# rdesc/autorally

Hardware: AMD Instinct MI355X
Metric: trajectory rollouts/s per MPPI solve (higher is better)
Workload: dtype f32

## Files before the change

autorally_amd/build.py:

```python
import os
import shutil
import subprocess
import sys
from concurrent.futures import ThreadPoolExecutor

HERE = os.path.dirname(os.path.abspath(__file__))
CSRC = os.path.join(HERE, "csrc")
LIB = os.path.join(HERE, "libmppi_hip.so")
SOURCES = ["mppi_abi.hip", "abi_forms.hip", "abi_pack.hip", "abi_solve.hip", "abi_host.hip", "abi_trace.hip", "rollout_mfma.hip", "rollout_multi.hip", "rollout_oct.hip", "rollout_row.hip", "rollout_row64.hip", "rollout_m44.hip", "rollout_lds44.hip", "rollout_lds128.hip", "rollout_lds16.hip", "rollout_fleet16.hip", "rollout_fleet_multi.hip", "rollout_glb16.hip", "rollout_glb44.hip", "rollout_valu.hip", "rollout_trace.hip", "ddp_fleet.hip", "nominal_fleet.hip", "solve_kernels.hip",
           "noise_mrg32k3a.hip", "rollout_bf.hip", "rollout_bf_row.hip", "ddp_feedback.cpp"]
HEADERS = ["abi_internal.hpp", "mppi_device.hpp", "mfma_net.hpp", "group_roles.hpp", "m44_core.hpp", "m44_group.hpp", "multi_group.hpp", "wave16_step.hpp", "wave16_image.hpp", "mppi_kernels.hpp", "noise_device.hpp", "ddp_feedback.hpp", "basis_funcs.hpp", "bf_device.hpp", "bf_row_device.hpp", "host_net.hpp", "tanhf_vec.hpp", "tanhf_scalar.hpp", "ddp_fleet_device.hpp", os.path.join("..", "..", "include", "mppi_hip.h")]
FLAGS = ["--offload-arch=gfx950", "-O3", "-ffp-contract=off", "-fPIC", "-std=c++17", "-Wall",
         "-Wno-unused-function", "-mllvm", "-amdgpu-mfma-vgpr-form", "-Xarch_host", "-mavx2", "-Xarch_host", "-mfma"]


EXTRA_FLAGS = {"rollout_row.hip": ["-mllvm", "-amdgpu-sched-strategy=max-ilp"],
               "rollout_row64.hip": ["-mllvm", "-amdgpu-sched-strategy=max-ilp"]}


def hipcc():
    for c in (os.environ.get("HIPCC"), shutil.which("hipcc"), "/opt/rocm/bin/hipcc"):
        if c and os.path.exists(c):
            return c
    raise RuntimeError("hipcc not found")


def _stale(target, deps):
    if not os.path.exists(target):
        return True
    t = os.path.getmtime(target)
    return any(os.path.getmtime(d) > t for d in deps)


def build(force=False, verbose=False):
    cc = hipcc()
    objdir = os.path.join(HERE, "build")
    os.makedirs(objdir, exist_ok=True)
    hdrs = [os.path.join(CSRC, h) for h in HEADERS]
    if not force and not _stale(LIB, [os.path.join(CSRC, s) for s in SOURCES] + hdrs):
        return LIB
    jobs = []
    objs = []
    for s in SOURCES:
        src = os.path.join(CSRC, s)
        obj = os.path.join(objdir, s.replace(".hip", ".o").replace(".cpp", ".o"))
        objs.append(obj)
        if force or _stale(obj, [src] + hdrs):
            jobs.append([cc] + FLAGS + EXTRA_FLAGS.get(s, []) + ["-c", src, "-o", obj])

    def run(cmd):
        if verbose:
            print(" ".join(cmd), file=sys.stderr)
        r = subprocess.run(cmd, capture_output=True, text=True)
        if r.returncode != 0:
            raise RuntimeError("hipcc failed:\n%s\n%s" % (" ".join(cmd), r.stderr))
        return r.stderr

    with ThreadPoolExecutor(max_workers=4) as ex:
        for warn in ex.map(run, jobs):
            if verbose and warn:
                print(warn, file=sys.stderr)
    if jobs or force or _stale(LIB, objs):
        run([cc, "--offload-arch=gfx950", "-shared", "-fPIC", "-o", LIB] + objs)
    return LIB


HOST = os.path.join(HERE, "host")
BIN = os.path.join(HERE, "bin")


def build_host(force=False):
    os.makedirs(BIN, exist_ok=True)
    cxx = shutil.which("g++") or "g++"
    hdrs = [os.path.join(HOST, h) for h in ("npz.hpp", "param_getter.hpp", "mppi_controller_hip.hpp",
                                            "run_control_loop.hpp", "path_integral_main.hpp")] + [os.path.join(CSRC, h) for h in ("basis_funcs.hpp", "host_net.hpp", "tanhf_vec.hpp")] + [os.path.join(HERE, "..", "include", "mppi_hip.h")]
    outs = []
    link = ["-L" + HERE, "-lmppi_hip", "-Wl,-rpath,$ORIGIN/.."]
    for name, libs in (("host_selftest", link), ("path_integral_nn", link), ("path_integral_bf", link)):
        src = os.path.join(HOST, name + ".cpp")
        out = os.path.join(BIN, name)
        outs.append(out)
        if force or _stale(out, [src] + hdrs + ([LIB] if libs else [])):
            cmd = [cxx, "-O2", "-mavx2", "-mfma", "-ffp-contract=off", "-std=c++17", "-Wall", "-DMPPI_NPZ_ZLIB", src, "-o", out] + libs + ["-lz", "-lpthread"]
            r = subprocess.run(cmd, capture_output=True, text=True)
            if r.returncode != 0:
                raise RuntimeError("host build failed:\n%s\n%s" % (" ".join(cmd), r.stderr))
    return outs


if __name__ == "__main__":
    print(build(force="--force" in sys.argv, verbose=True))
    print(build_host(force="--force" in sys.argv))
```

autorally_amd/csrc/abi_internal.hpp:

```cpp
#pragma once
#include "../../include/mppi_hip.h"

#include <hip/hip_runtime.h>

#include <chrono>
#include <cmath>
#include <cstdio>
#include <cstdlib>
#include <cstring>
#include <atomic>
#include <condition_variable>
#include <functional>
#include <mutex>
#include <new>
#include <thread>
#include <string>
#include <vector>

#include "mppi_kernels.hpp"
#include "ddp_feedback.hpp"
#include "basis_funcs.hpp"
#include "host_net.hpp"

namespace mppi_abi {
// ... 51 lines not shown
  NetDesc net{};
  bool mfma_ok = false;
  int hidden = 0, n_hidden = 0;
  mppi_abi::Pref pref = mppi_abi::Pref::Auto;
  mppi_abi::Form forced = mppi_abi::Form::Auto;
  bool multi_standalone_noise = false;
  int num_simds = 1024;
  hipStream_t stream = nullptr;
  hipStream_t order_stream = nullptr;
  int n_slots = 1;
  bool u_dirty = true;
  unsigned seq = 0;
  std::vector<float> sg_buf;
  bool basis = false;
  float ddp_Q[7] = {0.5f, 0.5f, 0.25f, 0.0f, 0.05f, 0.01f, 0.01f};
  float ddp_R[2] = {10.0f, 10.0f};
  float ddp_Qf[7] = {0, 0, 0, 0, 0, 0, 0};
  DdpResult ddp;
  bool have_ddp = false;
  int ddp_on_device = 0;
  int nominal_on_device = 0;
  hipStream_t batch_s = nullptr;
  unsigned *d_counter = nullptr;
  float *d_part = nullptr;
  unsigned long long *d_gx = nullptr;
  unsigned long long *d_min_cost = nullptr;
  unsigned min_cost_tag = 0;
  bool use_min_cost = true;
  unsigned long long *d_ug = nullptr;
  unsigned tail_epoch = 0, tail_poll_ticks = 2000000;
  float *d_res_map = nullptr;

  std::vector<float> U, hist, theta, map_rgba;
  HostNetFma hnet;
  int map_w = 0, map_h = 0;
  mppi_cost_params cost{};
  float r_c1[3] = {0, 0, 0}, r_c2[3] = {0, 0, 0}, trs[3] = {0, 0, 1};
  float u_lo[2] = {0, 0}, u_hi[2] = {0, 0};
  bool have_nn = false, have_map = false, have_cost = false;

  float *d_in = nullptr, *d_scal = nullptr;
  float *d_in_buf[2] = {nullptr, nullptr};
  int in_cur = 0;
  bool slid_valid = false;
  float *d_noise = nullptr, *d_stage = nullptr;
  float *d_gen[2] = {nullptr, nullptr};
  int gen_cur = 0;
  bool gen_async = false;
  bool prefetch_valid = false;
  float *v_buf = nullptr;
  hipStream_t gstream = nullptr;
  hipEvent_t ev_gen = nullptr, ev_s1 = nullptr;
  hipEvent_t ev_gt[2] = {nullptr, nullptr};
  bool gen_timed = false, gen_time_now = false;
  float *d_costs = nullptr, *d_w = nullptr;
  float *d_theta = nullptr, *d_wpack = nullptr, *d_map = nullptr;
  float *d_theta_s = nullptr;
  float *d_rowpack = nullptr;
  float *d_bfrowpack = nullptr;
  float *d_row64pack = nullptr;
  float *d_m44pack = nullptr;
  float *d_lds44pack = nullptr;
  float *d_lds128pack = nullptr;
  size_t lds128_bytes = 0;
  float *d_lds16pack = nullptr;
  size_t lds16_bytes = 0;
  mppi_abi::ArgBlock *fleet_one = nullptr;
  float *d_glb16pack = nullptr;
  size_t glb16_bytes = 0;
  int glb16_cap = -1;
  float *d_glb44pack = nullptr;
  size_t glb44_bytes = 0;
  int glb44_cap = -1;
  float *d_tracepack = nullptr;
  float *d_trace = nullptr;
  int *h_trace_ks = nullptr, *d_trace_ks = nullptr;
  int trace_chunk = 0;
  float solve_state[7] = {0, 0, 0, 0, 0, 0, 0};
  bool have_solve = false;
  bool have_weights = false;
  bool valu_reg_ok = false;
  double *d_invt = nullptr;
  uint32_t *d_rng[2] = {nullptr, nullptr};
  uint32_t *d_jump = nullptr, *d_sub = nullptr, *d_one = nullptr;
  int rng_cur = 0;
  int noise_L = 1, noise_C = 1;
  float *h_in = nullptr, *h_res = nullptr;
  int explicit_iters = 0;
  bool pending = false;
  bool pending_timed = false;
  bool pending_armed = false;
  float traj_cost = 0.0f, baseline = 0.0f, eta = 0.0f;

  int spin_budget = 0, fault_wave = 0;
  float *d_cap = nullptr;
  bool capture = false, cap_valid = false, cap_explicit = false;
  double wait_timeout_s = 30.0;
  unsigned *gate_cpu = nullptr, *d_gate = nullptr;
  bool gate_bar = false;
  bool chain = true;
  int gate_blk = 0;
  int armed = 0;
  unsigned arm_seq = 0;
  unsigned seq_floor = 0;
  int arm_in = 0;
  float *arm_vbuf = nullptr;
  bool arm_publish_only = false;
  int arm_n = 0;
  mppi_handle *arm_peers[4] = {nullptr, nullptr, nullptr, nullptr};
  hipStream_t arm_stream = nullptr;
  hipEvent_t ev_arm = nullptr;
  std::chrono::steady_clock::time_point arm_until;
  float *d_costs_alt = nullptr, *d_w_alt = nullptr;
  int launch_instances = 0;
  bool launch_gated = false;
  bool timed_out = false;
  bool no_result = false;
  bool timing = false;
  int timing_every = 1;
  unsigned timing_count = 0;
  std::vector<Events> ev;
  mppi_stage_times acc{};
  std::string err;
};

namespace mppi_abi {
using namespace mppi;


#define HIPCHK(h, call)                                                  \
  do {                                                                   \
    hipError_t e__ = (call);                                             \
    if (e__ != hipSuccess) return fail((h), MPPI_ERR_HIP, #call, e__);   \
  } while (0)
inline hipError_t ensure_device(int dev)
{
  int cur = -1;
  if (hipGetDevice(&cur) == hipSuccess && cur == dev) return hipSuccess;
  return hipSetDevice(dev);
}
#define OWN(h)                      \
  do {                              \
    int rc__ = own_stream(h);       \
    if (rc__) return rc__;          \
  } while (0)

int compute_k99(int K);
std::vector<float> pack_mfma_weights(const std::vector<float> &theta, int H, int NHID);
std::vector<float> pack_row_weights(const std::vector<float> &theta);
std::vector<float> pack_bf_row_weights(const std::vector<float> &W);
std::vector<float> pack_row64_weights(const std::vector<float> &theta, int NHID);
std::vector<float> pack_m44_weights(const std::vector<float> &theta, int NHID);
std::vector<float> pack_lds44_weights(const std::vector<float> &theta, const mppi::NetDesc &net);
std::vector<float> pack_lds128_weights(const std::vector<float> &theta, const mppi::NetDesc &net);
std::vector<float> pack_lds16_weights(const std::vector<float> &theta, const mppi::NetDesc &net);
std::vector<float> pack_glb16_weights(const std::vector<float> &theta, const mppi::NetDesc &net);
int upload_glb16_image(mppi_handle *h);
std::vector<float> pack_glb44_weights(const std::vector<float> &theta, const mppi::NetDesc &net);
int upload_glb44_image(mppi_handle *h);
std::vector<float> pack_trace_weights(const std::vector<float> &theta, const mppi::NetDesc &net);
int seed_device(mppi_handle *h, uint64_t seed, uint64_t offset);
int upload_rng_tables(mppi_handle *h);
bool use_mfma(const mppi_handle *h);
bool use_valu_reg(const mppi_handle *h);
Form form_of(const mppi_handle *h);
bool form_generator_noise(const mppi_handle *h);
// ... 62 lines not shown
```

autorally_amd/csrc/abi_pack.hip:

```cpp
#include "abi_internal.hpp"

using namespace mppi;
using namespace mppi_abi;

namespace mppi_abi {

constexpr uint64_t M1 = 4294967087ULL, M2 = 4294944443ULL;

struct Mat3 {
  uint32_t a[9];
};
Mat3 mat_mul(const Mat3 &A, const Mat3 &B, uint64_t m)
{
  Mat3 R;
  for (int i = 0; i < 3; i++)
    for (int j = 0; j < 3; j++) {
      uint64_t acc = 0;
      for (int k = 0; k < 3; k++) acc = (acc + (uint64_t)A.a[3 * i + k] * B.a[3 * k + j] % m) % m;
      R.a[3 * i + j] = (uint32_t)acc;
    }
  return R;
}
Mat3 mat_identity()
{
  Mat3 R{{1, 0, 0, 0, 1, 0, 0, 0, 1}};
  return R;
}
Mat3 mat_pow(Mat3 A, uint64_t e, uint64_t m)
{
  Mat3 R = mat_identity();
  while (e) {
    if (e & 1) R = mat_mul(R, A, m);
    A = mat_mul(A, A, m);
    e >>= 1;
  }
  return R;
}
Mat3 base_A1() { return Mat3{{0, 1, 0, 0, 0, 1, (uint32_t)(M1 - 810728ULL), 1403580u, 0}}; }
Mat3 base_A2() { return Mat3{{0, 1, 0, 0, 0, 1, (uint32_t)(M2 - 1370589ULL), 0, 527612u}}; }

int compute_k99(int K)
{
  const double thr = .99 * (double)K;
  int k = 0;
  while (k < K && !((double)k >= thr)) k++;
  return k;
}

std::vector<float> pack_mfma_weights(const std::vector<float> &theta, int H, int NHID)
{
  const int MT = H / 16, KSH = H / 4;
  const int nA0 = MT * 2, nAH = MT * KSH, nAL = KSH;
  const int nA = nA0 + (NHID - 1) * nAH + nAL;
  const int nBias = NHID * MT * 4 + 4;
  const int nTree = 4 * KSH + 1;
  std::vector<float> out((size_t)(nA + nBias + nTree) * 64, 0.0f);
  std::vector<int> wo, bo, nin, nout;
  int off = 0, prev = kNetIn;
  for (int l = 0; l <= NHID; l++) {
    const int no = (l < NHID) ? H : kNetOut;
    wo.push_back(off);
    bo.push_back(off + no * prev);
    nin.push_back(prev);
    nout.push_back(no);
    off += no * prev + no;
    prev = no;
  }
  for (int lane = 0; lane < 64; lane++) {
    const int row = lane & 15, kk = lane >> 4;
    const int gq = row >> 2, rq = row & 3;
    for (int m = 0; m < MT; m++)
      for (int s = 0; s < 2; s++) {
        const int n = 16 * m + 4 * rq + gq, kap = 4 * s + kk;
        out[(size_t)(m * 2 + s) * 64 + lane] = (kap < kNetIn) ? theta[wo[0] + n * kNetIn + kap] : 0.0f;
      }
    for (int l = 1; l < NHID; l++) {
      const int aoff = nA0 + (l - 1) * nAH;
      for (int m = 0; m < MT; m++)
        for (int s = 0; s < KSH; s++) {
          const int n = 16 * m + 4 * rq + gq, kap = 4 * s + kk;
          out[(size_t)(aoff + m * KSH + s) * 64 + lane] = theta[wo[l] + n * H + kap];
        }
    }
    {
      const int aoff = nA0 + (NHID - 1) * nAH;
      for (int s = 0; s < KSH; s++) {
        const int o = row & 3, kap = 4 * s + kk;
        out[(size_t)(aoff + s) * 64 + lane] = theta[wo[NHID] + o * H + kap];
      }
    }
    const int g = lane >> 4;
    for (int l = 0; l < NHID; l++)
      for (int m = 0; m < MT; m++)
        for (int r = 0; r < 4; r++)
          out[(size_t)(nA + l * MT * 4 + m * 4 + r) * 64 + lane] = theta[bo[l] + 16 * m + 4 * r + g];
    for (int r = 0; r < 4; r++) out[(size_t)(nA + NHID * MT * 4 + r) * 64 + lane] = theta[bo[NHID] + r];
    for (int s = 0; s < KSH; s++)
      for (int o = 0; o < 4; o++) out[(size_t)(nA + nBias + 4 * s + o) * 64 + lane] = theta[wo[NHID] + o * H + 4 * s + g];
    out[(size_t)(nA + nBias + 4 * KSH) * 64 + lane] = theta[bo[NHID] + g];
  }
  return out;
}

std::vector<float> pack_row_weights(const std::vector<float> &theta)
{
  const int H = 32;
  const float *W1 = theta.data(), *B1 = W1 + H * kNetIn, *W2 = B1 + H, *B2 = W2 + H * H, *W3 = B2 + H, *B3 = W3 + kNetOut * H;
  std::vector<float> out((size_t)row_pack_floats(), 0.0f);
  for (int p = 0; p < 16; p++) {
    const int j0 = 2 * p, j1 = 2 * p + 1, o0 = 2 * (p & 1), o1 = o0 + 1;
    auto entry = [&](int i) { return &out[((size_t)i * 16 + p) * 4]; };
    for (int i = 0; i < 3; i++) {
      float *e = entry(i);
      e[0] = W1[j0 * kNetIn + 2 * i]; e[1] = W1[j1 * kNetIn + 2 * i];
      e[2] = W1[j0 * kNetIn + 2 * i + 1]; e[3] = W1[j1 * kNetIn + 2 * i + 1];
    }
    for (int i = 0; i < H / 2; i++) {
      float *e = entry(3 + i), *f = entry(3 + H / 2 + i);
      e[0] = W2[j0 * H + 2 * i]; e[1] = W2[j1 * H + 2 * i]; e[2] = W2[j0 * H + 2 * i + 1]; e[3] = W2[j1 * H + 2 * i + 1];
      f[0] = W3[o0 * H + 2 * i]; f[1] = W3[o1 * H + 2 * i]; f[2] = W3[o0 * H + 2 * i + 1]; f[3] = W3[o1 * H + 2 * i + 1];
    }
    float *b = entry(35), *c = entry(36);
// ... 203 lines not shown
          for (int c = 0; c < 4; c++) {
            const int kap = 16 * mi + 4 * c + kk;
            if (kap < nin) wq[(block * 64 + l) * 4 + c] = W[(size_t)n * nin + kap];
          }
        }
      }
    p += (size_t)nout * nin + nout;
  }
  return out;
}
std::vector<float> pack_lds16_weights(const std::vector<float> &theta, const NetDesc &net)
{
  const size_t floats = (size_t)lds16_pack_floats(net);
  return floats ? pack_mfma16_image(theta, net, lds16_net_of(net), floats) : std::vector<float>();
}
std::vector<float> pack_glb16_weights(const std::vector<float> &theta, const NetDesc &net)
{
  const size_t floats = (size_t)glb16_pack_floats(net);
  return floats ? pack_mfma16_image(theta, net, glb16_net_of(net), floats) : std::vector<float>();
}
static int upload_named_image(mppi_handle *h, const std::vector<float> &pk, float *&d_img, size_t &bytes, const char *what)
{
  if (pk.empty() || h->theta.size() != (size_t)h->net.num_params) return fail(h, MPPI_ERR_INVALID, what);
  HIPCHK(h, hipSetDevice(h->cfg.device));
  if (!d_img) {
    bytes = pk.size() * sizeof(float);
    HIPCHK(h, hipMalloc(&d_img, bytes));
  }
  if (pk.size() * sizeof(float) != bytes) return fail(h, MPPI_ERR_INVALID, what);
  HIPCHK(h, hipStreamSynchronize(h->stream));
  HIPCHK(h, hipMemcpy(d_img, pk.data(), bytes, hipMemcpyHostToDevice));
  return MPPI_OK;
}
int upload_glb16_image(mppi_handle *h)
{
  return upload_named_image(h, pack_glb16_weights(h->theta, h->net), h->d_glb16pack, h->glb16_bytes, "glb16 image size");
}

std::vector<float> pack_glb44_weights(const std::vector<float> &theta, const NetDesc &net)
{
  std::vector<float> out((size_t)glb44_pack_floats(net), 0.0f);
  if (out.empty()) return out;
  const int n_w = net.n_layers - 1;
  const float *p = theta.data();
  int q0 = kGlb44BiasQuads;
  for (int j = 0; j < n_w; j++) {
    const int nin = net.layers[j], nout = net.layers[j + 1];
    const float *W = p, *B = p + (size_t)nout * nin;
    const bool last = j == n_w - 1;
    const int H = last ? 1 : (nout + 63) / 64;
    for (int h = 0; h < H; h++)
      for (int l = 0; l < 64; l++) {
        auto at = [&](int q, int c) -> float & { return out[((size_t)q * 64 + l) * 4 + c]; };
        const int n = last ? ((l & 15) == 0 ? (l >> 4) : -1) : (64 * h + l < nout ? 64 * h + l : -1);
        at(j, h) = last ? B[l >> 4] : (n >= 0 ? B[n] * kTanhScale : 0.0f);
        if (n >= 0)
          for (int k = 0; k < nin; k++) at(q0 + (k >> 2) * H + h, k & 3) = W[(size_t)n * nin + k];
      }
    q0 += ((nin + 3) / 4) * H;
    p += (size_t)nout * nin + nout;
  }
  return out;
}
int upload_glb44_image(mppi_handle *h)
{
  return upload_named_image(h, pack_glb44_weights(h->theta, h->net), h->d_glb44pack, h->glb44_bytes, "glb44 image size");
}

int seed_device(mppi_handle *h, uint64_t seed, uint64_t offset)
{
  uint32_t base[6] = {12345u, 12345u, 12345u, 12345u, 12345u, 12345u};
  if (seed != 0) {
    const uint32_t x1 = ((uint32_t)seed) ^ 0x55555555u;
    const uint32_t x2 = (uint32_t)((seed >> 32) ^ 0xAAAAAAAAu);
    base[0] = (uint32_t)((uint64_t)x1 * base[0] % M1);
    base[1] = (uint32_t)((uint64_t)x2 * base[1] % M1);
    base[2] = (uint32_t)((uint64_t)x1 * base[2] % M1);
    base[3] = (uint32_t)((uint64_t)x2 * base[3] % M2);
    base[4] = (uint32_t)((uint64_t)x1 * base[4] % M2);
    base[5] = (uint32_t)((uint64_t)x2 * base[5] % M2);
  }
  int sub_bits = 0;
  while ((1LL << sub_bits) < (long long)h->K) sub_bits++;
  HIPCHK(h, launch_noise_init(h->d_rng[0], h->K, base, h->d_sub, sub_bits, h->d_one, offset, h->stream));
  h->rng_cur = 0;
  h->cfg.seed = seed;
  return MPPI_OK;
}

int upload_rng_tables(mppi_handle *h)
{
  std::vector<uint32_t> sub(32 * 18), one(64 * 18), jump((size_t)h->noise_C * 18);
  Mat3 a1 = base_A1(), a2 = base_A2();
  for (int b = 0; b < 64; b++) {
    memcpy(&one[(size_t)b * 18], a1.a, 36);
    memcpy(&one[(size_t)b * 18 + 9], a2.a, 36);
    a1 = mat_mul(a1, a1, M1);
    a2 = mat_mul(a2, a2, M2);
  }
  for (int b = 64; b < 76; b++) {
    a1 = mat_mul(a1, a1, M1);
    a2 = mat_mul(a2, a2, M2);
  }
  for (int b = 0; b < 32; b++) {
    memcpy(&sub[(size_t)b * 18], a1.a, 36);
    memcpy(&sub[(size_t)b * 18 + 9], a2.a, 36);
    a1 = mat_mul(a1, a1, M1);
    a2 = mat_mul(a2, a2, M2);
  }
  const Mat3 j1 = mat_pow(base_A1(), 2ULL * (uint64_t)h->noise_L, M1);
  const Mat3 j2 = mat_pow(base_A2(), 2ULL * (uint64_t)h->noise_L, M2);
  Mat3 c1 = mat_identity(), c2 = mat_identity();
  for (int c = 0; c < h->noise_C; c++) {
    memcpy(&jump[(size_t)c * 18], c1.a, 36);
    memcpy(&jump[(size_t)c * 18 + 9], c2.a, 36);
    c1 = mat_mul(j1, c1, M1);
    c2 = mat_mul(j2, c2, M2);
  }
  HIPCHK(h, hipMemcpy(h->d_sub, sub.data(), sub.size() * 4, hipMemcpyHostToDevice));
  HIPCHK(h, hipMemcpy(h->d_one, one.data(), one.size() * 4, hipMemcpyHostToDevice));
  HIPCHK(h, hipMemcpy(h->d_jump, jump.data(), jump.size() * 4, hipMemcpyHostToDevice));
  return MPPI_OK;
}

std::vector<float> pack_trace_weights(const std::vector<float> &theta, const mppi::NetDesc &net)
{
  std::vector<float> img(theta.size());
  size_t off = 0;
  for (int l = 0; l + 1 < net.n_layers; l++) {
    const size_t nin = net.layers[l], nout = net.layers[l + 1];
    for (size_t j = 0; j < nout; j++)
      for (size_t k = 0; k < nin; k++) img[off + k * nout + j] = theta[off + j * nin + k];
    for (size_t j = 0; j < nout; j++) img[off + nin * nout + j] = theta[off + nin * nout + j];
    off += nin * nout + nout;
  }
  return img;
}

}
```

autorally_amd/csrc/abi_solve.hip:

```cpp
#include "abi_internal.hpp"

using namespace mppi;
using namespace mppi_abi;

namespace mppi_abi {

std::mutex g_batch_mu;
hipStream_t g_batch_stream[64] = {};
hipStream_t batch_stream(int device)
{
  if (device < 0 || device >= 64) return nullptr;
  std::lock_guard<std::mutex> lk(g_batch_mu);
  if (!g_batch_stream[device] &&
      hipStreamCreateWithFlags(&g_batch_stream[device], hipStreamNonBlocking) != hipSuccess)
    g_batch_stream[device] = nullptr;
  return g_batch_stream[device];
}

hipError_t arg_block_create(ArgBlock &b, size_t slot_bytes)
{
  b.slot = (slot_bytes + 255) & ~(size_t)255;
  hipError_t e = hipMalloc(reinterpret_cast<void **>(&b.d), b.slot);
  if (e == hipSuccess) e = hipHostMalloc(reinterpret_cast<void **>(&b.h), b.slot * ArgBlock::kRing, hipHostMallocDefault);
  for (int i = 0; i < ArgBlock::kRing && e == hipSuccess; i++) e = hipEventCreateWithFlags(&b.ev[i], hipEventDisableTiming);
// ... 53 lines not shown
{
  if (h->fleet_one) return MPPI_OK;
  HIPCHK(h, ensure_device(h->cfg.device));
  ArgBlock *b = new (std::nothrow) ArgBlock;
  if (!b) return fail(h, MPPI_ERR_HIP, "out of memory");
  const hipError_t e = arg_block_create(*b, sizeof(RolloutArgs));
  if (e != hipSuccess) {
    delete b;
    return fail(h, MPPI_ERR_HIP, "fleet form: argument block", e);
  }
  h->fleet_one = b;
  return MPPI_OK;
}

static hipError_t launch_rollout_fleet(const mppi_handle *h, const RolloutArgs *h_inst, const RolloutArgs *d_inst, int n, hipStream_t stream)
{
  if (h->forced == Form::FleetMulti4) return launch_rollout_fleet_multi(h->hidden, h->n_hidden, h_inst, d_inst, n, stream);
  return launch_rollout_fleet16(h->net, h_inst, d_inst, n, h->num_simds / 4, stream);
}

static hipError_t launch_rollout_fleet_one(mppi_handle *h, const RolloutArgs &a)
{
  if (!h->fleet_one) return hipErrorInvalidValue;
  unsigned char *host = nullptr;
  if (hipError_t e = arg_block_stage(*h->fleet_one, &host); e != hipSuccess) return e;
  memcpy(host, &a, sizeof(RolloutArgs));
  if (hipError_t e = arg_block_send(*h->fleet_one, sizeof(RolloutArgs), h->stream); e != hipSuccess) return e;
  return launch_rollout_fleet(h, &a, reinterpret_cast<const RolloutArgs *>(h->fleet_one->d), 1, h->stream);
}

void fill_cost_args(const mppi_handle *h, CostArgs &c)
{
  const mppi_cost_params &p = h->cost;
  c.desired_speed = p.desired_speed;
  c.speed_coeff = p.speed_coeff;
  c.track_coeff = p.track_coeff;
  c.max_slip_ang = p.max_slip_ang;
  c.slip_penalty = p.slip_penalty;
  c.track_slop = p.track_slop;
  c.crash_coeff = p.crash_coeff;
  c.steering_coeff = p.steering_coeff;
  c.throttle_coeff = p.throttle_coeff;
  c.boundary_threshold = p.boundary_threshold;
  c.crash_cost_discounted = (float)((1.0 - (double)p.discount) * (double)p.crash_coeff);
  c.l1_cost = p.l1_cost ? 1 : 0;
  for (int i = 0; i < 3; i++) {
    c.r_c1[i] = h->r_c1[i];
    c.r_c2[i] = h->r_c2[i];
    c.trs[i] = h->trs[i];
  }
  c.affine = (h->r_c1[2] == 0.0f && h->r_c2[2] == 0.0f && h->trs[2] == 1.0f) ? 1 : 0;
  const float n0 = h->cfg.exploration_std[0], n1 = h->cfg.exploration_std[1];
  const bool nu_ok = std::isfinite(n0) && std::isfinite(n1) && n0 * n0 > 0.0f && n1 * n1 > 0.0f &&
                     std::isfinite(n0 * n0) && std::isfinite(n1 * n1);
  c.need_control_cost = (p.steering_coeff != 0.0f || p.throttle_coeff != 0.0f || !nu_ok) ? 1 : 0;
  c.map_w = h->map_w;
  c.map_h = h->map_h;
  c.map = h->d_map;
}

void fill_rollout_args(const mppi_handle *h, const float *state, float *noise, RolloutArgs &a)
{
  for (int i = 0; i < kStateDim; i++) a.state[i] = state[i];
  a.U = h->d_in;
  a.noise = noise;
  a.costs = h->d_costs;
  const Form f = form_of(h);
  a.wpack = f == Form::BfRow ? h->d_bfrowpack : form_is_row(f) ? h->d_rowpack : form_is_row64(f) ? h->d_row64pack : (f == Form::M44 || f == Form::M44Chain) ? h->d_m44pack
            : f == Form::Lds44 ? h->d_lds44pack : f == Form::Lds128 ? h->d_lds128pack : (f == Form::Lds16 || f == Form::Fleet16) ? h->d_lds16pack : f == Form::Glb16 ? h->d_glb16pack : f == Form::Glb44 ? h->d_glb44pack : f == Form::ValuReg ? h->d_theta_s : (f == Form::ValuLds || h->basis) ? h->d_theta : h->d_wpack;
  a.inv_t = h->d_invt;
  a.K = h->K;
  a.T = h->T;
  a.opt_delay = h->cfg.optimization_stride;
  a.k99 = h->k99;
  for (int i = 0; i < 2; i++) {
    a.nu[i] = h->cfg.exploration_std[i];
    a.u_lo[i] = h->u_lo[i];
    a.u_hi[i] = h->u_hi[i];
  }
  a.dt = h->dt;
  a.negate_yaw_der = (h->cfg.negate_yaw_der || f == Form::BfRow) ? 1 : 0;
  a.rng_in = nullptr;
  a.rng_out = nullptr;
  a.inline_noise = 0;
  a.gate = nullptr;
  a.gate_seq = 0;
  a.gate_ticks = 10000000u;
  a.min_cost = nullptr;
  a.min_cost_tag = 0;
  a.spin_budget = h->fault_wave >= 32 ? 0 : h->spin_budget;
  a.fault_wave = h->fault_wave >= 32 ? 0 : h->fault_wave;
  fill_cost_args(h, a.cost);
}

static unsigned long long *min_cost_keys(const mppi_handle *h)
{
  const Form f = form_of(h);
  const bool publishes = f == Form::Multi2 || f == Form::Multi4 || f == Form::Multi4Tree || f == Form::FleetMulti4;
  return (h->use_min_cost && tail_is_stream(h->K) && publishes) ? h->d_min_cost : nullptr;
}

int tag_min_cost(mppi_handle *h, RolloutArgs &a, hipStream_t stream)
{
  h->min_cost_tag++;
  if (h->min_cost_tag == 0xFFFFFFFFu) {
    HIPCHK(h, hipMemsetAsync(h->d_min_cost, 0xFF, sizeof(unsigned long long) * kMinCostLines * kMinCostStride, stream));
    h->min_cost_tag = 1;
  }
  a.min_cost = min_cost_keys(h);
  a.min_cost_tag = h->min_cost_tag;
  return MPPI_OK;
}

int launch_rollout(mppi_handle *h, const RolloutArgs &a)
{
  const Form f = form_of(h);
  hipError_t e = hipSuccess;
  switch (f) {
    case Form::Bf1: case Form::Bf2: case Form::Bf3: e = launch_rollout_bf(a, form_bf_waves(f), h->stream); break;
    case Form::BfRow: e = launch_rollout_bf_row(a, h->stream); break;
    case Form::Multi2: case Form::Multi4: case Form::Multi4Tree:
      e = launch_rollout_multi(h->hidden, h->n_hidden, a, form_multi_nd(f), h->stream);
      break;
    case Form::Oct: e = launch_rollout_oct(h->hidden, h->n_hidden, a, h->stream); break;
    case Form::M44: e = launch_rollout_m44(h->hidden, h->n_hidden, a, true, h->stream); break;
    case Form::M44Chain: e = launch_rollout_m44(h->hidden, h->n_hidden, a, false, h->stream); break;
    case Form::Lds44: e = launch_rollout_lds44(h->net, a, h->stream); break;
    case Form::Lds128: e = launch_rollout_lds128(h->net, a, h->stream); break;
    case Form::Lds16: e = launch_rollout_lds16(h->net, a, h->num_simds / 4, h->stream); break;
    case Form::Fleet16: case Form::FleetMulti4: e = launch_rollout_fleet_one(h, a); break;
    case Form::Glb16: e = launch_rollout_glb16(h->net, a, h->num_simds / 4, h->glb16_cap, h->stream); break;
    case Form::Glb44: e = launch_rollout_glb44(h->net, a, h->glb44_cap, h->stream); break;
    case Form::Row64R16: e = launch_rollout_row64(h->hidden, h->n_hidden, a, 16, h->stream); break;
    case Form::Row: case Form::RowTree: e = launch_rollout_row(h->hidden, h->n_hidden, a, f == Form::RowTree, h->stream); break;
    case Form::Quad: case Form::Fused64: case Form::Fused256:
      e = launch_rollout_mfma(h->hidden, h->n_hidden, a, form_fused_threads(f), h->stream);
      break;
    case Form::ValuReg: e = launch_rollout_valu_reg(h->hidden, h->n_hidden, a, h->stream); break;
    default: e = launch_rollout_valu(h->net, a, h->stream); break;
  }
  if (e != hipSuccess) return fail(h, MPPI_ERR_HIP, "rollout launch", e);
  h->launch_instances = 1;
  h->launch_gated = a.gate != nullptr;
  return MPPI_OK;
}

int check_ready(mppi_handle *h)
{
  if (!h) return MPPI_ERR_INVALID;
  if (!h->have_nn) return fail(h, MPPI_ERR_STATE, "mppi_set_nn_params has not been called");
  if (!h->have_map) return fail(h, MPPI_ERR_STATE, "mppi_set_costmap has not been called");
  if (!h->have_cost) return fail(h, MPPI_ERR_STATE, "mppi_set_cost_params has not been called");
  return MPPI_OK;
}

int launch_generator(mppi_handle *h, float *dst)
{
  const bool timed = h->gen_time_now && !h->gen_timed;
  if (timed) HIPCHK(h, hipEventRecord(h->ev_gt[0], h->gstream));
  HIPCHK(h, launch_noise(h->d_rng[h->rng_cur], h->d_rng[1 - h->rng_cur], h->d_jump, h->K, h->T, h->noise_L,
                         h->noise_C, dst, h->gstream));
  if (timed) {
    HIPCHK(h, hipEventRecord(h->ev_gt[1], h->gstream));
    h->gen_timed = true;
  }
  h->rng_cur = 1 - h->rng_cur;
  HIPCHK(h, hipEventRecord(h->ev_gen, h->gstream));
  return MPPI_OK;
}

int acquire_noise(mppi_handle *h, float **buf_out)
{
  if (!h->gen_async) {
    h->gen_cur = 1 - h->gen_cur;
    float *dst = h->d_gen[h->gen_cur];
    HIPCHK(h, launch_noise(h->d_rng[h->rng_cur], h->d_rng[1 - h->rng_cur], h->d_jump, h->K, h->T, h->noise_L,
                           h->noise_C, dst, h->stream));
    h->rng_cur = 1 - h->rng_cur;
    *buf_out = dst;
    return MPPI_OK;
  }
  if (!h->prefetch_valid) {
    HIPCHK(h, hipEventRecord(h->ev_s1, h->stream));
    HIPCHK(h, hipStreamWaitEvent(h->gstream, h->ev_s1, 0));
    int rc = launch_generator(h, h->d_gen[1 - h->gen_cur]);
    if (rc) return rc;
  }
  h->prefetch_valid = false;
  h->gen_cur = 1 - h->gen_cur;
  HIPCHK(h, hipStreamWaitEvent(h->stream, h->ev_gen, 0));
  *buf_out = h->d_gen[h->gen_cur];
  return MPPI_OK;
}

bool gen_beside_rollout(const mppi_handle *h)
{
  static const int forced = [] { const char *e = getenv("MPPI_GEN_BESIDE"); return e ? (atoi(e) != 0 ? 1 : 0) : -1; }();
  if (forced >= 0) return forced == 1;
  if (h->K / kRolloutsPerWave <= h->num_simds) return true;
  if (h->hidden >= 64) return true;
  return h->K / 64 <= 2 * (h->num_simds / 4);
}

int prefetch_noise(mppi_handle *h)
{
  if (h->pending) return fail(h, MPPI_ERR_STATE, "prefetch with a solve pending");
  if (!gen_beside_rollout(h)) HIPCHK(h, hipStreamWaitEvent(h->gstream, h->ev_s1, 0));
  int rc = launch_generator(h, h->d_gen[1 - h->gen_cur]);
  if (rc) return rc;
  h->prefetch_valid = true;
  return MPPI_OK;
}

static unsigned next_seq(const mppi_handle *h)
{
  return (h->seq_floor - h->seq < 0x80000000u ? h->seq_floor : h->seq) + 1;
}

static void next_tail_epoch(mppi_handle *h)
{
  if (++h->tail_epoch == 0) h->tail_epoch = 1;
}

static void use_inline_noise(mppi_handle *h, RolloutArgs &a)
{
  a.inline_noise = 1;
  a.rng_in = h->d_rng[h->rng_cur];
  a.rng_out = h->d_rng[1 - h->rng_cur];
  h->rng_cur = 1 - h->rng_cur;
}

static int hand_over(mppi_handle *h, hipStream_t batch)
{
  if (h->order_stream == batch) return MPPI_OK;
  hipError_t e = hipStreamSynchronize(work_stream(h));
  if (e == hipSuccess) e = hipStreamSynchronize(h->gstream);
  if (e != hipSuccess) return fail(h, MPPI_ERR_HIP, "stream hand-over to the batch stream", e);
  h->order_stream = batch;
  return MPPI_OK;
}

int upload_controls_if_dirty(mppi_handle *h, hipStream_t stream)
{
  if (!h->u_dirty) return MPPI_OK;
  memcpy(h->h_in, h->U.data(), sizeof(float) * 2 * (size_t)h->T);
  memcpy(h->h_in + 2 * h->T, h->hist.data(), sizeof(float) * 4);
  HIPCHK(h, hipMemcpyAsync(h->d_in, h->h_in, sizeof(float) * (2 * (size_t)h->T + 4), hipMemcpyHostToDevice,
                           stream));
  h->u_dirty = false;
  return MPPI_OK;
}

#ifdef MPPI_HOSTPROF
static double hp_acc[8] = {0}, hp_n = 0;
static std::chrono::steady_clock::time_point hp_seen;
#define HP(i, t0) hp_acc[i] += std::chrono::duration<double, std::micro>(std::chrono::steady_clock::now() - (t0)).count()
#endif

void savgol_host(mppi_handle *h, const float *src, int stride, int off1)
{
  const int T = h->T;
  std::vector<float> &X = h->sg_buf;
  X.resize((size_t)(T + 4) * 2);
  for (int j = 0; j < 4; j++) X[j] = h->hist[j];
  for (int t = 0; t < T; t++) {
    X[(t + 2) * 2 + 0] = src[stride * t + 0];
    X[(t + 2) * 2 + 1] = src[stride * t + off1];
  }
  for (int r = T + 2; r < T + 4; r++)
    for (int j = 0; j < 2; j++) X[r * 2 + j] = X[(T + 1) * 2 + j];
  const float f0 = -3.0f / 35.0f, f1 = 12.0f / 35.0f, f2 = 17.0f / 35.0f;
  for (int i = 0; i < 2 * T; i++) {
    float acc = f0 * X[i];
    float p = f1 * X[i + 2];
    acc = acc + p;
    p = f2 * X[i + 4];
    acc = acc + p;
    p = f1 * X[i + 6];
    acc = acc + p;
    p = f0 * X[i + 8];
    acc = acc + p;
    h->U[i] = acc;
  }
}

int recover_timed_out(mppi_handle *h)
{
  if (!h->timed_out) return MPPI_OK;
  const hipError_t q = hipStreamQuery(work_stream(h));
  if (q == hipErrorNotReady) return fail(h, MPPI_ERR_HIP, "an earlier solve timed out and its device work has not finished yet");
  if (q != hipSuccess) return fail(h, MPPI_ERR_HIP, "an earlier solve timed out; hipStreamQuery", q);
  h->timed_out = false;
  return MPPI_OK;
}

int wait_pending(mppi_handle *h)
{
  if (!h->pending) return recover_timed_out(h);
  const volatile unsigned *words = reinterpret_cast<const volatile unsigned *>(h->h_res);
  const int n_entries = h->T + 2;
  const auto t0 = std::chrono::steady_clock::now();
  unsigned long spins = 0;
  double next_query_s = 0.01;
  int next = 0;
  auto give_up = [&](const char *what, bool timed_out) {
    h->pending = false;
    h->pending_armed = false;
    h->pending_timed = false;
    h->u_dirty = true;
    h->slid_valid = false;
    h->timed_out = timed_out;
    h->no_result = true;
// ... 60 lines not shown
      h->gen_timed = false;
      float gms = 0.0f;
      HIPCHK(h, hipEventSynchronize(h->ev_gt[1]));
      if (hipEventElapsedTime(&gms, h->ev_gt[0], h->ev_gt[1]) == hipSuccess && gms > 0.0f) h->acc.noise_ms += gms;
    }
    h->acc.n_solves += 1;
  }
  return MPPI_OK;
}

bool wants_slid_copy(const mppi_handle *h)
{
  return h->cfg.optimization_stride >= 1 && h->cfg.optimization_stride < h->T;
}

TailLaunch tail_launch(const mppi_handle *h, const float *V, bool last)
{
  TailLaunch l;
  l.costs = h->d_costs; l.V = V; l.U = h->d_in; l.hist = h->d_in + 2 * h->T; l.w = h->d_w; l.scal = h->d_scal;
  l.res = h->d_res_map; l.counter = h->d_counter;
  l.K = h->K; l.T = h->T; l.gamma = h->cfg.gamma; l.last_iter = last ? 1 : 0; l.seq = h->seq;
  l.slid = (last && wants_slid_copy(h)) ? h->d_in_buf[1 - h->in_cur] : nullptr;
  l.slide_stride = h->cfg.optimization_stride;
  l.init0 = h->cfg.init_control[0]; l.init1 = h->cfg.init_control[1];
  l.ug = h->d_ug;
  l.gx = h->d_gx; l.gpart = reinterpret_cast<unsigned long long *>(h->d_part);
  l.epoch = h->tail_epoch;
  l.fault = h->fault_wave >= 32 ? h->fault_wave : 0;
  l.poll_ticks = (l.fault && h->spin_budget > 0) ? (unsigned)h->spin_budget * 100u : h->tail_poll_ticks;
  l.min_cost = min_cost_keys(h);
  l.min_cost_tag = h->min_cost_tag;
  return l;
}

static bool arm_usable(const mppi_handle *h);
static int open_armed(mppi_handle *h, const float *state);

int enqueue_solve(mppi_handle *h, const float *state)
{
#ifdef MPPI_HOSTPROF
  const auto hp_t0 = std::chrono::steady_clock::now();
  if (hp_n > 0) hp_acc[0] += std::chrono::duration<double, std::micro>(hp_t0 - hp_seen).count();
#endif
  int rc = check_ready(h);
  if (rc) return rc;
  if (!state) return fail(h, MPPI_ERR_INVALID, "state is NULL");
  rc = recover_timed_out(h);
  if (rc) return rc;
  rc = wait_pending(h);
  if (h->armed) {
    if (rc == MPPI_OK && h->arm_n == 0 && arm_usable(h)) return open_armed(h, state);
    const int drc = solve_ahead_disarm(h);
    if (rc == MPPI_OK) rc = drc;
  }
  if (rc) return rc;
  const int K = h->K, T = h->T, iters = h->cfg.num_iters;
  if (h->explicit_iters > 0 && h->explicit_iters != iters)
    return fail(h, MPPI_ERR_STATE, "explicit noise holds a different number of iterations");
  OWN(h);
  rc = upload_controls_if_dirty(h, h->stream);
  if (rc) return rc;
  const bool timed = h->timing && (h->timing_count++ % (unsigned)h->timing_every) == 0;
  const bool explicit_noise = h->explicit_iters > 0;
  const size_t slot_sz = (size_t)K * T * 2;
  h->seq = next_seq(h);
  forget_solve_state(h);
  for (int it = 0; it < iters; it++) {
    Events *ev = timed ? &h->ev[it] : nullptr;
    if (ev) HIPCHK(h, hipEventRecord(ev->e[0], h->stream));
    const bool inline_noise = !explicit_noise && !h->prefetch_valid && has_noise_wave(h);
    float *noise = h->d_noise + (size_t)(explicit_noise ? it : 0) * slot_sz;
    if (!explicit_noise && !inline_noise) {
      rc = acquire_noise(h, &noise);
      if (rc) return rc;
    } else if (inline_noise) {
      noise = h->d_gen[h->gen_cur];
    }
    h->v_buf = noise;
    if (ev) HIPCHK(h, hipEventRecord(ev->e[1], h->stream));
    RolloutArgs a;
    fill_rollout_args(h, state, noise, a);
    rc = tag_min_cost(h, a, h->stream);
    if (rc) return rc;
    if (inline_noise) use_inline_noise(h, a);
#ifdef MPPI_HOSTPROF
    HP(1, hp_t0);
    const auto hp_t1 = std::chrono::steady_clock::now();
#endif
    if (ev) { tl_kernel_start = ev->e[4]; tl_kernel_stop = ev->e[5]; }
    rc = launch_rollout(h, a);
    tl_kernel_start = tl_kernel_stop = nullptr;
    if (rc) return rc;
#ifdef MPPI_HOSTPROF
    HP(2, hp_t1);
    const auto hp_t2 = std::chrono::steady_clock::now();
#endif
    const bool prefetch = h->gen_async && iters == 1 && !explicit_noise && !has_noise_wave(h) && !h->prefetch_valid;
    if (prefetch) HIPCHK(h, hipEventRecord(h->ev_s1, h->stream));
    if (ev) HIPCHK(h, hipEventRecord(ev->e[2], h->stream));
    const bool last = (it == iters - 1);
    const bool want_slid = last && wants_slid_copy(h);
    next_tail_epoch(h);
    HIPCHK(h, launch_solve_tail(tail_launch(h, noise, last), h->stream));
    if (last) h->slid_valid = want_slid;
    if (h->capture) {
      float *c = h->d_cap + (size_t)it * (2 * (size_t)T + K);
      if (!last) HIPCHK(h, hipMemcpyAsync(c, h->d_in, sizeof(float) * 2 * (size_t)T, hipMemcpyDeviceToDevice, h->stream));
      HIPCHK(h, hipMemcpyAsync(c + 2 * (size_t)T, h->d_costs, sizeof(float) * (size_t)K, hipMemcpyDeviceToDevice, h->stream));
    }
    if (prefetch) {
      h->gen_time_now = timed;
      rc = prefetch_noise(h);
      h->gen_time_now = false;
      if (rc) return rc;
    }
#ifdef MPPI_HOSTPROF
    HP(3, hp_t2);
    hp_n += 1;
    if ((long)hp_n % 2000 == 0)
      fprintf(stderr, "hostprof n=%.0f: seen->enqueue %.2f us, entry->launch %.2f, rollout launch %.2f, tail launch %.2f, poll->smoothed %.2f\n",
              hp_n, hp_acc[0] / hp_n, hp_acc[1] / hp_n, hp_acc[2] / hp_n, hp_acc[3] / hp_n, hp_acc[4] / hp_n);
#endif
    if (ev) HIPCHK(h, hipEventRecord(ev->e[3], h->stream));
  }
  h->explicit_iters = 0;
  h->pending = true;
  note_solve_state(h, state, true);
  h->pending_timed = timed;
  h->cap_valid = h->capture;
  h->cap_explicit = explicit_noise;
  return MPPI_OK;
}


static int arm_kind(const mppi_handle *h)
{
  const Form f = form_of(h);
  if (!(h->d_gate != nullptr && wants_slid_copy(h) && h->cfg.num_iters == 1 && !h->timing && !h->capture &&
        h->explicit_iters == 0 && (!h->basis || f == Form::BfRow) && h->fault_wave == 0 && h->have_nn && h->have_map && h->have_cost && !h->timed_out))
    return 0;
  if (form_has_gate(f) && has_noise_wave(h) && !h->prefetch_valid) return 1;
  if (f == Form::Multi4Tree && h->forced == Form::Auto && !has_noise_wave(h) && h->gen_async && gen_beside_rollout(h)) return 2;
  return 0;
}

static void write_gate_payload(mppi_handle *h, const float *state)
{
  unsigned *g = gate_host(h);
  const int T = h->T;
  memcpy(g + kGateUOffset, h->U.data(), sizeof(float) * 2 * (size_t)T);
  memcpy(g + gate_hist_offset(T), h->hist.data(), sizeof(float) * 4);
  for (int r = 0; r < kGateReplicas; r++) memcpy(g + 16 * r, state, sizeof(float) * kStateDim);
}

static void write_gate_word(mppi_handle *h, unsigned word)
{
  unsigned *g = gate_host(h);
  asm volatile("" ::: "memory");
  __builtin_ia32_sfence();
  for (int r = 0; r < kGateReplicas; r++) __atomic_store_n(g + 16 * r + 7, word, __ATOMIC_RELAXED);
  __builtin_ia32_sfence();
}

static unsigned arm_ticks(double max_wait_s) { return (unsigned)(max_wait_s * 1e8); }
static std::chrono::steady_clock::time_point arm_deadline(double max_wait_s)
{
  const double open_s = 0.9 * max_wait_s - 50e-6;
  return std::chrono::steady_clock::now() + std::chrono::nanoseconds((long long)((open_s > 0.0 ? open_s : 0.0) * 1e9));
}

static void armed_args(mppi_handle *h, float *noise, RolloutArgs &a, TailLaunch &l, double max_wait_s)
{
  static const float no_state[kStateDim] = {0, 0, 0, 0, 0, 0, 0};
  fill_rollout_args(h, no_state, noise, a);
  a.costs = h->d_costs_alt;
  a.U = reinterpret_cast<const float *>(gate_dev(h)) + kGateUOffset;
  a.gate = gate_dev(h);
  a.gate_seq = h->arm_seq;
  a.gate_ticks = arm_ticks(max_wait_s);
  l = tail_launch(h, noise, true);
  l.costs = h->d_costs_alt;
  l.w = h->d_w_alt;
  l.seq = h->arm_seq;
  l.hist = reinterpret_cast<const float *>(gate_dev(h)) + gate_hist_offset(h->T);
  l.U = h->d_in;
  l.hist_out = h->d_in + 2 * h->T;
  l.slid = h->d_in_buf[1 - h->in_cur];
}

static void mark_armed(mppi_handle *h, int kind, float *vbuf, hipStream_t stream, double max_wait_s, bool publish_only)
{
  h->armed = kind;
  h->arm_in = h->in_cur;
  h->arm_vbuf = vbuf;
  h->arm_stream = stream;
  h->arm_until = arm_deadline(max_wait_s);
  h->arm_n = 0;
  h->arm_publish_only = publish_only;
  h->u_dirty = true;
  h->slid_valid = false;
}

static int arm_handle(mppi_handle *h, int kind, hipStream_t stream, double max_wait_s, bool publish_only, bool mark,
                      RolloutArgs &a, TailLaunch &l)
{
  h->arm_seq = next_seq(h);
  h->gate_blk ^= 1;
  float *noise = h->d_gen[1 - h->gen_cur];
  if (kind == 2) {
    int rc = acquire_noise(h, &noise);
    if (rc) return rc;
  }
  if (mark) HIPCHK(h, hipEventRecord(h->ev_arm, stream));
  armed_args(h, noise, a, l, max_wait_s);
  int rc = tag_min_cost(h, a, stream);
  if (rc) return rc;
  l.min_cost_tag = h->min_cost_tag;
  if (publish_only) {
    l.no_device_copy = 1;
    l.slid = nullptr;
  }
  if (kind == 1) use_inline_noise(h, a);
  next_tail_epoch(h);
  l.epoch = h->tail_epoch;
  mark_armed(h, kind, noise, stream, max_wait_s, publish_only);
  return MPPI_OK;
}

static int arm_one(mppi_handle *h, double max_wait_s, bool publish_only, bool mark)
{
  const int kind = arm_kind(h);
  if (!kind) return fail(h, MPPI_ERR_UNSUPPORTED, "this handle's form / configuration has no gated form (mppi_arm)");
  OWN(h);
  RolloutArgs a;
  TailLaunch l;
  int rc = arm_handle(h, kind, h->stream, max_wait_s, publish_only, mark, a, l);
  if (rc) return rc;
  rc = launch_rollout(h, a);
  if (rc == MPPI_OK) {
    const hipError_t e = launch_solve_tail(l, h->stream);
    if (e != hipSuccess) rc = fail(h, MPPI_ERR_HIP, "armed tail launch", e);
  }
  if (rc) (void)solve_ahead_disarm(h);
  return rc;
}

static int disarm_one(mppi_handle *h)
{
  if (!h->armed) return MPPI_OK;
  const int kind = h->armed;
  h->armed = 0;
  h->arm_n = 0;
  write_gate_word(h, h->arm_seq | kGateCancel);
  h->seq_floor = h->arm_seq;
  h->u_dirty = true;
  h->slid_valid = false;
  h->order_stream = h->arm_stream;
  if (kind == 1) {
    h->rng_cur = 1 - h->rng_cur;
    return MPPI_OK;
  }
  HIPCHK(h, ensure_device(h->cfg.device));
  h->gen_cur = 1 - h->gen_cur;
  h->rng_cur = 1 - h->rng_cur;
  HIPCHK(h, hipEventRecord(h->ev_s1, h->arm_stream));
  HIPCHK(h, hipStreamWaitEvent(h->gstream, h->ev_s1, 0));
  int rc = launch_generator(h, h->d_gen[1 - h->gen_cur]);
  if (rc) return rc;
  h->prefetch_valid = true;
  return MPPI_OK;
}

int solve_ahead_disarm(mppi_handle *h)
{
  if (!h || !h->armed) return MPPI_OK;
  if (h->arm_n > 0) {
    mppi_handle *peers[kMaxBatch];
    const int n = h->arm_n;
    for (int i = 0; i < n; i++) peers[i] = h->arm_peers[i];
    int rc = MPPI_OK;
    for (int i = 0; i < n; i++) {
      const int r = disarm_one(peers[i]);
      if (r && !rc) rc = r;
    }
    return rc;
  }
  return disarm_one(h);
}

static bool arm_usable(const mppi_handle *h)
{
  if (std::chrono::steady_clock::now() >= h->arm_until) return false;
  const volatile unsigned *words = reinterpret_cast<const volatile unsigned *>(h->h_res);
  const unsigned s1 = __atomic_load_n(words + 1, __ATOMIC_ACQUIRE), s3 = __atomic_load_n(words + 4 * (h->T + 1) + 1, __ATOMIC_ACQUIRE);
  return s1 != h->arm_seq && s3 != h->arm_seq;
}

static int open_armed(mppi_handle *h, const float *state)
{
  const int kind = h->armed;
  h->armed = 0;
  h->arm_n = 0;
  h->seq = h->arm_seq;
  note_solve_state(h, state, true);
  write_gate_payload(h, state);
// ... 110 lines not shown
    together = form_ok && ci.affine == c0.affine && ctrl_ok &&
               h->cfg.device == h0->cfg.device && h->cfg.num_iters == h0->cfg.num_iters &&
               h->K <= 4096 && !h->timing && !h->capture && !h->prefetch_valid && h->have_nn && h->have_map && h->have_cost;
    waves += (h->basis && f != Form::BfRow) ? 3 * (h->K / 64) : 4 * (h->K / kRolloutsPerWave);
  }
  return together && waves <= h0->num_simds;
}

static bool fleet_together(mppi_handle *const *hs, int n)
{
  if (n < 2 || n > kMaxFleet) return false;
  const mppi_handle *h0 = hs[0];
  CostArgs c0;
  fill_cost_args(h0, c0);
  for (int i = 0; i < n; i++) {
    const mppi_handle *h = hs[i];
    if (h->basis || (h0->forced != Form::Fleet16 && h0->forced != Form::FleetMulti4) || h->forced != h0->forced || h->fleet_one == nullptr || h->cfg.device != h0->cfg.device || h->cfg.num_iters != h0->cfg.num_iters) return false;
    if (h->net.n_layers != h0->net.n_layers) return false;
    for (int l = 0; l < h->net.n_layers; l++)
      if (h->net.layers[l] != h0->net.layers[l]) return false;
    CostArgs ci;
    fill_cost_args(h, ci);
    if (ci.affine != c0.affine || ci.need_control_cost != c0.need_control_cost) return false;
    if (h->K > 4096 || h->K % 64 != 0 || h->timing || h->capture || h->prefetch_valid || h->armed || !h->have_nn || !h->have_map || !h->have_cost) return false;
  }
  return true;
}

static int enqueue_fleet(mppi_handle *const *hs, const float *states, int n)
{
  mppi_handle *h0 = hs[0];
  HIPCHK(h0, ensure_device(h0->cfg.device));
  if (!h0->batch_s) h0->batch_s = batch_stream(h0->cfg.device);
  const hipStream_t S = h0->batch_s;
  if (!S) return fail(h0, MPPI_ERR_HIP, "no batch stream");
  FleetBlock *fb = fleet_block(h0->cfg.device);
  if (!fb) return fail(h0, MPPI_ERR_HIP, "no argument block for the fleet");
  const int iters = h0->cfg.num_iters;
  for (int i = 0; i < n; i++) {
    mppi_handle *h = hs[i];
    int rc = recover_timed_out(h);
    if (rc == MPPI_OK) rc = wait_pending(h);
    if (rc) return rc;
    if (h->explicit_iters > 0 && h->explicit_iters != iters)
      return fail(h, MPPI_ERR_STATE, "explicit noise holds a different number of iterations");
  }
  auto poison = [&](int rc_) {
    for (int i = 0; i < n; i++) {
      hs[i]->slid_valid = false;
      hs[i]->u_dirty = true;
      hs[i]->pending = false;
    }
    return rc_;
  };
  std::lock_guard<std::mutex> lk(fb->mu);
  for (int i = 0; i < n; i++) {
    mppi_handle *h = hs[i];
    int rc = hand_over(h, S);
    if (rc == MPPI_OK) rc = upload_controls_if_dirty(h, S);
    if (rc) return poison(rc);
    h->seq = next_seq(h);
    forget_solve_state(h);
  }
  TailLaunch tl[kMaxFleet];
  for (int it = 0; it < iters; it++) {
    const bool last = (it == iters - 1);
    unsigned char *host = nullptr;
    hipError_t e = arg_block_stage(fb->args, &host);
    if (e != hipSuccess) return poison(fail(h0, MPPI_ERR_HIP, "fleet argument block", e));
    RolloutArgs *ra = reinterpret_cast<RolloutArgs *>(host);
    NoiseFleetDesc *nd = reinterpret_cast<NoiseFleetDesc *>(host + fleet_noise_offset(n));
    for (int i = 0; i < n; i++) {
      mppi_handle *h = hs[i];
      const bool explicit_noise = h->explicit_iters > 0;
      float *noise;
      nd[i] = NoiseFleetDesc{};
      if (explicit_noise) {
        noise = h->d_noise + (size_t)it * ((size_t)h->K * h->T * 2);
      } else {
        h->gen_cur = 1 - h->gen_cur;
        noise = h->d_gen[h->gen_cur];
        nd[i] = NoiseFleetDesc{h->d_rng[h->rng_cur], h->d_rng[1 - h->rng_cur], h->d_jump, noise, h->K, h->T, h->noise_L, h->noise_C};
        h->rng_cur = 1 - h->rng_cur;
      }
      h->v_buf = noise;
      fill_rollout_args(h, states + (size_t)MPPI_STATE_DIM * i, noise, ra[i]);
      if (int trc = tag_min_cost(h, ra[i], S)) return poison(trc);
      next_tail_epoch(h);
      tl[i] = tail_launch(h, noise, last);
      if (last) h->slid_valid = wants_slid_copy(h);
    }
    fill_solve_tail_fleet(host + fleet_tail_offset(n), tl, n);
    e = arg_block_send(fb->args, fleet_bytes(n), S);
    const unsigned char *dev = fb->args.d;
    if (e == hipSuccess) e = launch_noise_fleet(nd, reinterpret_cast<const NoiseFleetDesc *>(dev + fleet_noise_offset(n)), n, S);
    if (e == hipSuccess)
      e = launch_rollout_fleet(h0, ra, reinterpret_cast<const RolloutArgs *>(dev), n, S);
    if (e == hipSuccess) e = launch_solve_tail_fleet(tl, n, dev + fleet_tail_offset(n), S);
    if (e != hipSuccess) return poison(fail(h0, MPPI_ERR_HIP, "fleet launch", e));
    for (int i = 0; i < n; i++) {
      hs[i]->launch_instances = n;
      hs[i]->launch_gated = false;
    }
  }
  for (int i = 0; i < n; i++) {
    hs[i]->explicit_iters = 0;
    hs[i]->pending = true;
    note_solve_state(hs[i], states + (size_t)MPPI_STATE_DIM * i, true);
    hs[i]->pending_timed = false;
  }
  return MPPI_OK;
}

static bool armed_as_batch(mppi_handle *const *hs, int n)
{
  for (int i = 0; i < n; i++) {
    if (!hs[i]->armed || hs[i]->arm_n != n) return false;
    for (int q = 0; q < n; q++)
      if (hs[i]->arm_peers[q] != hs[q]) return false;
  }
  return true;
}

}

extern "C" {

int mppi_compute_control_async(mppi_handle *h, const float state[MPPI_STATE_DIM])
{
  if (!h) return MPPI_ERR_INVALID;
  HIPCHK(h, ensure_device(h->cfg.device));
  return enqueue_solve(h, state);
}

int mppi_synchronize(mppi_handle *h)
{
  if (!h) return MPPI_ERR_INVALID;
  return wait_pending(h);
}

int mppi_compute_control(mppi_handle *h, const float state[MPPI_STATE_DIM])
{
  int rc = mppi_compute_control_async(h, state);
  if (rc) return rc;
  return mppi_synchronize(h);
}

int mppi_compute_control_batch_async(mppi_handle *const *hs, const float *states, int n)
{
  if (!hs || !states || n < 1) return MPPI_ERR_INVALID;
#ifdef MPPI_HOSTPROF
  static double hb[8] = {0}; static double hbn = 0; static std::chrono::steady_clock::time_point hb_prev_end;
  auto hb_t = std::chrono::steady_clock::now();
  if (hbn > 0) hb[0] += std::chrono::duration<double, std::micro>(hb_t - hb_prev_end).count();
#define HB(i) do { auto n__ = std::chrono::steady_clock::now(); hb[i] += std::chrono::duration<double, std::micro>(n__ - hb_t).count(); hb_t = n__; } while (0)
#else
#define HB(i) do { } while (0)
#endif
  for (int i = 0; i < n; i++) {
    if (!hs[i]) return MPPI_ERR_INVALID;
    for (int q = 0; q < i; q++)
      if (hs[q] == hs[i]) return fail(hs[i], MPPI_ERR_INVALID, "the same handle twice in one batch");
  }
  if (n == 2 && g_host_threads.load(std::memory_order_relaxed) >= 2) host_helper_arm();
  if (armed_as_batch(hs, n)) {
    int rc = MPPI_OK;
// ... 3 lines not shown
      if (rc == MPPI_OK) rc = check_ready(h);
      if (rc == MPPI_OK) rc = recover_timed_out(h);
      if (rc == MPPI_OK) rc = wait_pending(h);
      usable = usable && arm_usable(h);
    }
    if (rc == MPPI_OK && usable) {
      for (int i = 0; i < n; i++) {
        const int orc = open_armed(hs[i], states + (size_t)MPPI_STATE_DIM * i);
        if (orc && !rc) rc = orc;
      }
      return rc;
    }
    const int drc = solve_ahead_disarm(hs[0]);
    if (rc) return rc;
    if (drc) return drc;
  }
  const bool together = batch_together(hs, n);
  for (int i = 0; i < n; i++) {
    if (hs[i]->armed && (hs[i]->arm_n > 0 || together)) {
      const int drc = solve_ahead_disarm(hs[i]);
      if (drc) return drc;
    }
  }
  mppi_handle *h0 = hs[0];
  if (!together && fleet_together(hs, n)) return enqueue_fleet(hs, states, n);
  if (!together && n >= 2) {
    bool all_fleet = h0->forced == Form::Fleet16 || h0->forced == Form::FleetMulti4;
    for (int i = 0; i < n; i++) all_fleet = all_fleet && hs[i]->forced == h0->forced;
    for (int i = 0; i < n && all_fleet; i++)
      if (const int rc = check_ready(hs[i])) return rc;
  }
  if (!together) {
    for (int i = 0; i < n; i++) {
      const int rc = mppi_compute_control_async(hs[i], states + (size_t)MPPI_STATE_DIM * i);
      if (rc) return rc;
    }
    return MPPI_OK;
  }
  HB(1);
  HIPCHK(h0, ensure_device(h0->cfg.device));
  if (!h0->batch_s) h0->batch_s = batch_stream(h0->cfg.device);
  const hipStream_t S = h0->batch_s;
  if (!S) return fail(h0, MPPI_ERR_HIP, "no batch stream");
  const int iters = h0->cfg.num_iters;
  HB(2);
  for (int i = 0; i < n; i++) {
    mppi_handle *h = hs[i];
    int rc = recover_timed_out(h);
    if (rc == MPPI_OK) rc = wait_pending(h);
    if (rc) return rc;
    if (h->explicit_iters > 0 && h->explicit_iters != iters)
      return fail(h, MPPI_ERR_STATE, "explicit noise holds a different number of iterations");
  }
  auto poison = [&](int rc_) {
    for (int i = 0; i < n; i++) {
      hs[i]->slid_valid = false;
      hs[i]->u_dirty = true;
      hs[i]->pending = false;
    }
    return rc_;
  };
  HB(3);
  for (int i = 0; i < n; i++) {
    mppi_handle *h = hs[i];
    int rc = hand_over(h, S);
    if (rc == MPPI_OK) rc = upload_controls_if_dirty(h, S);
    if (rc) return poison(rc);
    h->seq = next_seq(h);
    forget_solve_state(h);
  }
  for (int it = 0; it < iters; it++) {
    QuadBatchArgs qb;
    TailLaunch tl[kMaxBatch];
    qb.n = n;
    const bool last = (it == iters - 1);
    for (int i = 0; i < n; i++) {
      mppi_handle *h = hs[i];
      const bool explicit_noise = h->explicit_iters > 0;
      float *noise = explicit_noise ? h->d_noise + (size_t)it * ((size_t)h->K * h->T * 2) : h->d_gen[h->gen_cur];
      h->v_buf = noise;
      RolloutArgs &a = qb.inst[i];
      fill_rollout_args(h, states + (size_t)MPPI_STATE_DIM * i, noise, a);
      if (int trc = tag_min_cost(h, a, S)) return trc;
      if (!explicit_noise) use_inline_noise(h, a);
      tl[i] = tail_launch(h, noise, last);
      if (last) h->slid_valid = wants_slid_copy(h);
    }
    for (int i = n; i < kMaxBatch; i++) qb.inst[i] = qb.inst[0];
    HB(4);
    hipError_t e = launch_rollout_batch(hs, n, qb, false, S);
    HB(5);
    if (e == hipSuccess) e = launch_solve_tail_batch(tl, n, S);
    HB(6);
    if (e != hipSuccess) return poison(fail(h0, MPPI_ERR_HIP, "batched launch", e));
  }
  for (int i = 0; i < n; i++) {
    hs[i]->explicit_iters = 0;
    hs[i]->pending = true;
    note_solve_state(hs[i], states + (size_t)MPPI_STATE_DIM * i, true);
    hs[i]->pending_timed = false;
  }
#ifdef MPPI_HOSTPROF
  hbn += 1;
  hb_prev_end = std::chrono::steady_clock::now();
  if (((long)hbn % 1000) == 0)
    fprintf(stderr, "hostprof batch (us per call, %.0f calls): between calls %.2f | decide %.2f | device + stream %.2f | wait_pending %.2f | upload+args %.2f | rollout launch %.2f | tail launch %.2f\n",
            hbn, hb[0] / hbn, hb[1] / hbn, hb[2] / hbn, hb[3] / hbn, hb[4] / hbn, hb[5] / hbn, hb[6] / hbn);
#endif
  return MPPI_OK;
}

int mppi_compute_control_batch(mppi_handle *const *hs, const float *states, int n)
{
  int rc = mppi_compute_control_batch_async(hs, states, n);
  for (int i = 0; i < n && rc == MPPI_OK; i++) rc = mppi_synchronize(hs[i]);
  return rc;
}

int mppi_control_ticks_batch(mppi_handle *const *hs, const float *states, int n, int n_ticks, int stride)
{
  if (!hs || !states || n < 1 || n_ticks < 0 || stride < 0) return MPPI_ERR_INVALID;
  for (int t = 0; t < n_ticks; t++) {
    int rc = mppi_compute_control_batch(hs, states, n);
    if (rc) return rc;
    for (int i = 0; i < n && stride > 0; i++) {
      rc = mppi_slide_control_seq(hs[i], stride);
      if (rc) return rc;
    }
  }
  return MPPI_OK;
}

int mppi_control_ticks(mppi_handle *h, const float state[MPPI_STATE_DIM], int n_ticks, int stride)
{
  if (!h || n_ticks < 0 || stride < 0) return MPPI_ERR_INVALID;
  DISARM(h);
  if (state && h->chain && n_ticks >= 2 && stride == h->cfg.optimization_stride && arm_kind(h)) {
    HIPCHK(h, ensure_device(h->cfg.device));
    int rc = enqueue_solve(h, state);
    for (int i = 0; i < n_ticks && rc == MPPI_OK; i++) {
      const bool ahead = i + 1 < n_ticks;
      if (ahead) rc = arm_one(h, 0.1, i + 2 < n_ticks, false);
      if (rc == MPPI_OK) rc = wait_pending(h);
      if (rc == MPPI_OK) rc = mppi_slide_control_seq(h, stride);
      if (rc == MPPI_OK && ahead) rc = enqueue_solve(h, state);
    }
    if (rc) (void)solve_ahead_disarm(h);
    return rc;
  }
  for (int i = 0; i < n_ticks; i++) {
    int rc = mppi_compute_control(h, state);
    if (rc) return rc;
    if (stride > 0) {
      rc = mppi_slide_control_seq(h, stride);
      if (rc) return rc;
    }
  }
  return MPPI_OK;
}

int mppi_get_results(mppi_handle *h, float *U, float *traj_cost, float *costs, float *weights)
{
  if (!h) return MPPI_ERR_INVALID;
  int rc = mppi_synchronize(h);
  if (rc) return rc;
  if (h->no_result) return fail(h, MPPI_ERR_HIP, "the last solve timed out: no result");
  if (U) memcpy(U, h->U.data(), sizeof(float) * 2 * (size_t)h->T);
  if (traj_cost) *traj_cost = h->traj_cost;
  if ((costs || weights) && h->armed) {
    HIPCHK(h, hipSetDevice(h->cfg.device));
    HIPCHK(h, hipEventSynchronize(h->ev_arm));
  } else if (costs || weights) {
    HIPCHK(h, hipSetDevice(h->cfg.device));
    OWN(h);
    HIPCHK(h, hipStreamSynchronize(h->stream));
  }
  if (costs) HIPCHK(h, hipMemcpy(costs, h->d_costs, sizeof(float) * h->K, hipMemcpyDeviceToHost));
  if (weights) HIPCHK(h, hipMemcpy(weights, h->d_w, sizeof(float) * h->K, hipMemcpyDeviceToHost));
  return MPPI_OK;
}

int mppi_get_applied_controls(mppi_handle *h, float *V, size_t n)
{
  if (!h || !V) return MPPI_ERR_INVALID;
  const size_t slot = (size_t)h->K * h->T * 2;
  if (n != slot) return fail(h, MPPI_ERR_INVALID, "n != K*T*2");
  int rc = mppi_synchronize(h);
  if (rc) return rc;
  if (h->no_result) return fail(h, MPPI_ERR_HIP, "the last solve timed out: no result");
  HIPCHK(h, hipSetDevice(h->cfg.device));
  if (h->armed) {
    HIPCHK(h, hipStreamWaitEvent(h->gstream, h->ev_arm, 0));
    HIPCHK(h, launch_tk_to_kt(h->v_buf, h->d_stage, h->K, h->T, h->gstream));
    HIPCHK(h, hipMemcpyAsync(V, h->d_stage, slot * sizeof(float), hipMemcpyDeviceToHost, h->gstream));
    HIPCHK(h, hipStreamSynchronize(h->gstream));
    return MPPI_OK;
  }
  OWN(h);
  HIPCHK(h, launch_tk_to_kt(h->v_buf, h->d_stage, h->K, h->T, h->stream));
  HIPCHK(h, hipMemcpyAsync(V, h->d_stage, slot * sizeof(float), hipMemcpyDeviceToHost, h->stream));
  HIPCHK(h, hipStreamSynchronize(h->stream));
  return MPPI_OK;
}

int mppi_rollout_only(mppi_handle *h, const float state[MPPI_STATE_DIM], float *costs)
{
  int rc = check_ready(h);
  if (rc) return rc;
  if (!state || !costs) return fail(h, MPPI_ERR_INVALID, "NULL argument");
  DISARM(h);
  HIPCHK(h, hipSetDevice(h->cfg.device));
  rc = recover_timed_out(h);
  if (rc) return rc;
  rc = mppi_synchronize(h);
  if (rc) return rc;
  OWN(h);
  rc = upload_controls_if_dirty(h, h->stream);
  if (rc) return rc;
  const bool explicit_noise = h->explicit_iters > 0;
  const bool inline_noise = !explicit_noise && !h->prefetch_valid && has_noise_wave(h);
  float *noise = h->d_noise;
  if (!explicit_noise && !inline_noise) {
    rc = acquire_noise(h, &noise);
    if (rc) return rc;
  } else if (inline_noise) {
    noise = h->d_gen[h->gen_cur];
  }
  h->explicit_iters = 0;
  forget_solve_state(h);
  h->v_buf = noise;
  RolloutArgs a;
  fill_rollout_args(h, state, noise, a);
  if (inline_noise) use_inline_noise(h, a);
  rc = launch_rollout(h, a);
  if (rc) return rc;
  note_solve_state(h, state, false);
  HIPCHK(h, hipMemcpyAsync(costs, h->d_costs, sizeof(float) * h->K, hipMemcpyDeviceToHost, h->stream));
  HIPCHK(h, hipStreamSynchronize(h->stream));
  return MPPI_OK;
}

int mppi_debug_capture_iterations(mppi_handle *h, int on)
{
  if (!h) return MPPI_ERR_INVALID;
  DISARM(h);
  int rc = mppi_synchronize(h);
  if (rc) return rc;
  if (on && !h->d_cap) {
    HIPCHK(h, hipSetDevice(h->cfg.device));
    HIPCHK(h, hipMalloc(&h->d_cap, sizeof(float) * (size_t)h->cfg.num_iters * (2 * (size_t)h->T + h->K)));
  }
  h->capture = on != 0;
  h->cap_valid = false;
  return MPPI_OK;
}

int mppi_debug_get_iterations(mppi_handle *h, float *U_raw, float *costs, float *V)
{
  if (!h) return MPPI_ERR_INVALID;
  int rc = mppi_synchronize(h);
  if (rc) return rc;
  if (!h->cap_valid) return fail(h, MPPI_ERR_STATE, "no captured solve (mppi_debug_capture_iterations, then a solve on this handle alone)");
  if (V && !h->cap_explicit) return fail(h, MPPI_ERR_STATE, "applied controls of every iteration exist for explicit-noise solves only");
  const int iters = h->cfg.num_iters, T = h->T, K = h->K;
  HIPCHK(h, hipSetDevice(h->cfg.device));
  OWN(h);
  HIPCHK(h, hipStreamSynchronize(h->stream));
  const size_t rec = 2 * (size_t)T + K;
  std::vector<float> buf((size_t)iters * rec);
  HIPCHK(h, hipMemcpy(buf.data(), h->d_cap, sizeof(float) * buf.size(), hipMemcpyDeviceToHost));
  for (int it = 0; it < iters; it++) {
    if (U_raw) {
      float *u = U_raw + (size_t)it * 2 * T;
      if (it < iters - 1) memcpy(u, buf.data() + (size_t)it * rec, sizeof(float) * 2 * (size_t)T);
      else for (int t = 0; t < T; t++) { u[2 * t] = h->h_res[4 * t]; u[2 * t + 1] = h->h_res[4 * t + 2]; }
    }
    if (costs) memcpy(costs + (size_t)it * K, buf.data() + (size_t)it * rec + 2 * (size_t)T, sizeof(float) * (size_t)K);
    if (V) {
      const size_t slot = (size_t)K * T * 2;
      HIPCHK(h, launch_tk_to_kt(h->d_noise + (size_t)it * slot, h->d_stage, K, T, h->stream));
      HIPCHK(h, hipMemcpyAsync(V + (size_t)it * slot, h->d_stage, slot * sizeof(float), hipMemcpyDeviceToHost, h->stream));
      HIPCHK(h, hipStreamSynchronize(h->stream));
    }
  }
  return MPPI_OK;
}

int mppi_arm(mppi_handle *h, double max_wait_s)
{
  if (!h || !(max_wait_s > 0.0 && max_wait_s <= 0.1)) return MPPI_ERR_INVALID;
  if (h->armed && h->arm_n == 0) return MPPI_OK;
  DISARM(h);
  HIPCHK(h, ensure_device(h->cfg.device));
  return arm_one(h, max_wait_s, false, true);
}

int mppi_arm_batch(mppi_handle *const *hs, int n, double max_wait_s)
{
  if (!hs || n < 1 || n > 64 || !(max_wait_s > 0.0 && max_wait_s <= 0.1)) return MPPI_ERR_INVALID;
  for (int i = 0; i < n; i++) {
    if (!hs[i]) return MPPI_ERR_INVALID;
    for (int q = 0; q < i; q++)
      if (hs[q] == hs[i]) return fail(hs[i], MPPI_ERR_INVALID, "the same handle twice in one batch");
  }
  if (n >= 2 && armed_as_batch(hs, n)) return MPPI_OK;
  for (int i = 0; i < n; i++)
    if (hs[i]->armed && (hs[i]->arm_n > 0 || n >= 2)) DISARM(hs[i]);
  if (n >= 2) {
    for (int i = 0; i < n; i++) {
      int rc = check_ready(hs[i]);
      if (rc) return rc;
    }
    if (batch_together(hs, n)) return arm_together(hs, n, max_wait_s);
  }
  int out = MPPI_OK;
  for (int i = 0; i < n; i++) {
// ... 35 lines not shown
```

autorally_amd/csrc/group_roles.hpp:

```cpp
#pragma once

#include "mppi_device.hpp"
#include "noise_device.hpp"

namespace mppi {

constexpr int kGRing = 16;
constexpr int kGCtlChunk = 4;

template <class SH>
struct GroupRoles {
  static constexpr int kPose = SH::NW, kCost = SH::NW + 1, kCtl = SH::NW + 2, kRng = SH::NW + 3;
  static constexpr int kWaves = SH::NW + 4;
  static_assert(kWaves <= (int)(sizeof(SH::fin) / sizeof(int)), "fin[]");
  static_assert(SH::kR == 16 || SH::kR == 8, "rollouts per group");
};
template <class SH>
__device__ __forceinline__ int group_j(int slot) { return slot & (SH::kR - 1); }
template <class SH>
__device__ __forceinline__ bool group_real(int slot) { return slot < SH::kR; }

template <class SH>
__device__ __forceinline__ int group_seq_min(SH &sh)
{
  int m = lds_peek(lds_addr(&sh.xseq[0][0]));
#pragma unroll
  for (int w = 1; w < SH::NW; w++) m = min(m, lds_peek(lds_addr(&sh.xseq[w][0])));
  return m;
}

struct MrgHalf {
  uint32_t s0, s1, s2;
};
__device__ __forceinline__ uint32_t fold_m(uint64_t x, uint32_t C, uint32_t m)
{
  x = (x >> 32) * C + (x & 0xffffffffULL);
  x = (x >> 32) * C + (x & 0xffffffffULL);
  x = (x >> 32) * C + (x & 0xffffffffULL);
  if (x >= m) x -= m;
  return (uint32_t)x;
}
template <class SH>
__device__ __forceinline__ MrgHalf group_rng_load(const RolloutArgs &a)
{
  const int lane = threadIdx.x & 63;
  const int j = group_j<SH>((lane >> 1) & 15), c = lane & 1;
  const int k = (int)blockIdx.x * SH::kR + j;
  const int K = a.K;
  MrgHalf g{0, 0, 0};
  if (a.inline_noise != 0 && lane < 2 * kRolloutsPerWave) {
    g.s0 = a.rng_in[(3 * c) * K + k]; g.s1 = a.rng_in[(3 * c + 1) * K + k]; g.s2 = a.rng_in[(3 * c + 2) * K + k];
  }
  return g;
}
template <class SH, bool PRE = false>
__device__ __forceinline__ void group_rng_wave(const RolloutArgs &a, SH &sh, const MrgHalf pre = MrgHalf{0, 0, 0})
{
  using R = GroupRoles<SH>;
  const int lane = threadIdx.x & 63;
  const int j = group_j<SH>((lane >> 1) & 15), c = lane & 1;
  const int k = (int)blockIdx.x * SH::kR + j;
  const int K = a.K, T = a.T;
  const bool active = lane < 2 * kRolloutsPerWave;
  const bool real = lane < 2 * SH::kR;
  int budget = spin_budget_init(a.spin_budget, T, a.fault_wave == R::kRng + 1);
  if (a.inline_noise != 0) {
    const uint32_t m = c ? (uint32_t)kM2 : (uint32_t)kM1, C = c ? kC2 : kC1;
    const uint32_t A = c ? (uint32_t)kA21 : (uint32_t)kA12, Bn = c ? (uint32_t)kA23N : (uint32_t)kA13N;
    MrgHalf g{0, 0, 0};
    if constexpr (PRE) {
      g = pre;
    } else if (active) {
      g.s0 = a.rng_in[(3 * c) * K + k]; g.s1 = a.rng_in[(3 * c + 1) * K + k]; g.s2 = a.rng_in[(3 * c + 2) * K + k];
    }
    const uint32_t a_ctl = lds_addr(&sh.ctl_pub[0]);
    const uint32_t a_mypub = lds_addr(&sh.rng_pub[lane]);
    int seen = 0;
    for (int t = 0; t < T; t++) {
      float2 e = make_float2(0.5f, 0.5f);
#ifdef MPPI_DIAG_NORNG
      e = make_float2(0.25f + 0.001f * (float)t, 0.5f);
#else
#pragma unroll
      for (int d = 0; d < 2; d++) {
        const uint32_t p = fold_m((uint64_t)A * (c ? g.s2 : g.s1) + (uint64_t)Bn * (m - g.s0), C, m);
        g.s0 = g.s1; g.s1 = g.s2; g.s2 = p;
        const uint32_t p2 = (uint32_t)__builtin_amdgcn_mov_dpp((int)p, 0xB1, 0xF, 0xF, false);
        uint32_t z = (p >= p2) ? p - p2 : p + (uint32_t)kM1 - p2;
        if (z == 0) z = (uint32_t)kM1;
        const float u = (float)z * 0x1p-32f;
        if (d == 0) e.x = u; else e.y = u;
      }
#endif
      const int need = t - kGRing + 1;
      while (seen < need && --budget > 0) {
        seen = lds_peek(a_ctl);
        if (seen < need) __builtin_amdgcn_s_sleep(2);
      }
      if (active && c == 0) *reinterpret_cast<float2 *>(&sh.eps[t & (kGRing - 1)][j][0]) = e;
      lds_publish(a_mypub, t + 1);
    }
    if (real) {
      a.rng_out[(3 * c) * K + k] = g.s0; a.rng_out[(3 * c + 1) * K + k] = g.s1; a.rng_out[(3 * c + 2) * K + k] = g.s2;
    }
  }
  spin_finish(budget, lds_addr(&sh.fail[0]), lds_addr(&sh.fin[R::kRng]));
}

template <class SH>
__device__ __forceinline__ void group_control_wave(const RolloutArgs &a, SH &sh, const uint32_t a_gate_open = 0)
{
  using R = GroupRoles<SH>;
  constexpr int NSW = SH::NSW;
  static_assert(kGCtlChunk == 4 && kGRing >= 2 * kGCtlChunk, "four steps per iteration, lanes 16 q + j");
  const int lane = threadIdx.x & 63;
  const int j = group_j<SH>(lane & 15), q = lane >> 4;
  const bool real = group_real<SH>(lane & 15);
  const int k = (int)blockIdx.x * SH::kR + j;
  const int K = a.K, T = a.T;
  const bool inl = a.inline_noise != 0;
  float2 *const noise = reinterpret_cast<float2 *>(a.noise);
  const float2 *const Useq = reinterpret_cast<const float2 *>(a.U);
  const bool noise_free_k = (k == 0);
  const bool pure_noise_k = (k >= a.k99);
  const uint32_t a_cd = lds_addr(&sh.cost_done[0]);
  const uint32_t a_mypub = lds_addr(&sh.ctl_pub[lane]);
  const uint32_t a_rng = lds_addr(&sh.rng_pub[0]);
  int budget = spin_budget_init(a.spin_budget, T, a.fault_wave == R::kCtl + 1);
  const bool gated = a_gate_open != 0;
  if (gated)
    while (lds_peek(a_gate_open) == 0 && --budget > 0) __builtin_amdgcn_s_sleep(1);
  int seen_x = 0, seen_c = 0, seen_r = 0;
  for (int t0 = 0, n = 1; t0 < T; t0 += n, n = kGCtlChunk) {
    const int t = t0 + q;
    const bool live = (t < T) & (q < n);
    const int tl = live ? t : T - 1;
    float2 Ut;
    if (gated) {
      const unsigned long long ub = __hip_atomic_load(reinterpret_cast<const unsigned long long *>(Useq + tl), __ATOMIC_RELAXED, __HIP_MEMORY_SCOPE_SYSTEM);
      Ut = make_float2(__uint_as_float((unsigned)ub), __uint_as_float((unsigned)(ub >> 32)));
    } else {
      Ut = Useq[tl];
    }
    float2 e = (live && !inl) ? noise[(size_t)tl * K + k] : make_float2(0.0f, 0.0f);
    const int tm = min(t0 + n, T) - 1;
    const int need_x = (tm >= kGRing) ? (tm - kGRing) * NSW + 1 : 0;
    const int need_c = tm - kGRing + 1;
    while ((seen_x < need_x || seen_c < need_c) && --budget > 0) {
      seen_x = group_seq_min(sh);
      seen_c = lds_peek(a_cd);
      if (seen_x < need_x || seen_c < need_c) __builtin_amdgcn_s_sleep(2);
    }
    if (inl) {
      while (seen_r < tm + 1 && --budget > 0) {
        seen_r = lds_peek(a_rng);
        if (seen_r < tm + 1) __builtin_amdgcn_s_sleep(1);
      }
#ifdef MPPI_DIAG_NOBM
      e = *reinterpret_cast<const float2 *>(&sh.eps[tl & (kGRing - 1)][j][0]);
#else
      e = box_muller(*reinterpret_cast<const float2 *>(&sh.eps[tl & (kGRing - 1)][j][0]));
#endif
    }
    if (live) {
      const bool nf = noise_free_k | (t < a.opt_delay);
      const float n0 = e.x * a.nu[0], n1 = e.y * a.nu[1];
      const float du0 = nf ? 0.0f : n0, du1 = nf ? 0.0f : n1;
      float u0 = nf ? Ut.x : (pure_noise_k ? n0 : Ut.x + n0);
      float u1 = nf ? Ut.y : (pure_noise_k ? n1 : Ut.y + n1);
      if (real) noise[(size_t)t * K + k] = make_float2(u0, u1);
      u0 = clampf(u0, a.u_lo[0], a.u_hi[0]);
      u1 = clampf(u1, a.u_lo[1], a.u_hi[1]);
      const int slot = t & (kGRing - 1);
      sh.ctl_b1[slot][j] = u0;
      sh.ctl_b1[slot][kRolloutsPerWave + j] = u1;
      *reinterpret_cast<float4 *>(&sh.ctl_rec[slot][j][0]) = make_float4(u0, u1, du0, du1);
    }
    lds_publish(a_mypub, tm + 1);
  }
  spin_finish(budget, lds_addr(&sh.fail[0]), lds_addr(&sh.fin[R::kCtl]));
}

template <class SH, bool AFFINE>
__device__ __forceinline__ void group_pose_wave(const RolloutArgs &a, SH &sh)
{
  using R = GroupRoles<SH>;
  constexpr int NSW = SH::NSW;
  static_assert(SH::kR == 16, "one step per iteration: 16-rollout groups only");
  const int lane = threadIdx.x & 63;
  const int j = lane & 15;
  const int T = a.T;
  const uint32_t a_seq0 = lds_addr(&sh.xseq[0][0]);
  const uint32_t a_cd = lds_addr(&sh.cost_done[0]);
  const uint32_t a_mypub = lds_addr(&sh.pose_pub[lane]);
  float x = a.state[0], y = a.state[1], yaw = a.state[2];
  int budget = spin_budget_init(a.spin_budget, T, a.fault_wave == R::kPose + 1), seen = 0, cdone = 0;
  float tf_p = 0.0f, tb_p = 0.0f;
  for (int t = 0; t <= T; t++) {
    float tf = 0.0f, tb = 0.0f;
    if (t < T) {
      const int need = t * NSW + 1;
      while (seen < need && --budget > 0) {
        seen = SH::kRecByAll ? group_seq_min(sh) : lds_peek(a_seq0);
        if (seen < need) __builtin_amdgcn_s_sleep(1);
      }
      const float4 r0 = *reinterpret_cast<const float4 *>(&sh.rec[t & (kGRing - 1)][j][0]);
      float spsi, cpsi;
#ifdef MPPI_DIAG_NOPOSE
      spsi = 0.0f; cpsi = 1.0f; tf = x; tb = y;
#else
      sincos_fast(yaw, spsi, cpsi);
      const float st[3] = {x, y, yaw};
      track_fetch<AFFINE>(a.cost, st, cpsi, spsi, tf, tb);
#endif
      const float sd0 = fmaf(cpsi, r0.y, -(spsi * r0.z));
      const float sd1 = fmaf(spsi, r0.y, cpsi * r0.z);
      const float sd2 = a.negate_yaw_der ? -r0.w : r0.w;
      x = fmaf(sd0, a.dt, x);
      y = fmaf(sd1, a.dt, y);
      yaw = fmaf(sd2, a.dt, yaw);
    }
    if (t > 0) {
      while (cdone < t - kGRing && --budget > 0) cdone = lds_peek(a_cd);
      if (lane < kRolloutsPerWave) *reinterpret_cast<float2 *>(&sh.tex[(t - 1) & (kGRing - 1)][lane][0]) = make_float2(tf_p, tb_p);
      lds_publish(a_mypub, t);
    }
    tf_p = tf; tb_p = tb;
  }
  spin_finish(budget, lds_addr(&sh.fail[0]), lds_addr(&sh.fin[R::kPose]));
}

template <int Q>
__device__ __forceinline__ float quad_bc(float v)
{
  return __int_as_float(__builtin_amdgcn_mov_dpp(__float_as_int(v), Q * 0x55, 0xF, 0xF, false));
}
__device__ __forceinline__ void quad_chain(float v, float d, float dt, int q, float &vq, float &v_out)
{
  const float v1 = fmaf(quad_bc<0>(d), dt, v);
  const float v2 = fmaf(quad_bc<1>(d), dt, v1);
  const float v3 = fmaf(quad_bc<2>(d), dt, v2);
  v_out = fmaf(quad_bc<3>(d), dt, v3);
  const float lo = (q == 0) ? v : v1, hi = (q == 2) ? v2 : v3;
  vq = (q < 2) ? lo : hi;
// ... 177 lines not shown
```

autorally_amd/csrc/m44_group.hpp:

```cpp
#pragma once
#include "group_roles.hpp"
#include "m44_core.hpp"
#include "mppi_kernels.hpp"

namespace mppi {

struct M44GroupShared {
  static constexpr int NW = 4;
  static constexpr int NSW = 1;
  static constexpr int kR = 16;
  static constexpr bool kRecByAll = true;
  int xseq[NW][64];
  float rec[kGRing][kRolloutsPerWave][4];
  int cost_done[64];
  float ctl_b1[kGRing][64];
  float ctl_rec[kGRing][kRolloutsPerWave][4];
  int ctl_pub[64];
  float tex[kGRing][kRolloutsPerWave][2];
  int pose_pub[64];
  float eps[kGRing][kRolloutsPerWave][2];
  int rng_pub[64];
  int fail[4];
  int fin[8];
  float gstate[8];
  int gate_open[8];
  float dump[NW][64 * kGRing];
};

constexpr size_t kM44GroupImageOffset = (sizeof(M44GroupShared) + 15) & ~(size_t)15;
extern __shared__ __attribute__((aligned(16))) unsigned char m44_group_smem[];
struct M44LayerList {
  int n_layers;
  int layers[8];
};
inline M44LayerList m44_layer_list_of(const NetDesc &net)
{
  M44LayerList nd;
  nd.n_layers = net.n_layers;
  for (int i = 0; i < 8; i++) nd.layers[i] = net.layers[i];
  return nd;
}

template <bool GATED>
struct M44Wave {
  typedef const volatile int __attribute__((address_space(3))) *lds_int_p;
  typedef const volatile f32x2 __attribute__((address_space(3))) *lds_f2_p;
  static constexpr int kSlotF2 = kRolloutsPerWave * 2;
  static constexpr uint32_t kRecStride = sizeof(float) * kRolloutsPerWave * 4;
  static_assert(kRecStride == sizeof(float) * 64, "dump rows move along with the record's ring slot");
  uint32_t a_myseq, a_rec0;
  lds_int_p p_pub;
  lds_f2_p p_u;
  int budget, sn, cp_v;
  float sv;
  f32x2 un;

  __device__ __forceinline__ M44Wave(const RolloutArgs &a, M44GroupShared &sh, const int w)
  {
    const int lane = threadIdx.x & 63;
    const int row = lane >> 4;
    const int jr = 4 * w + (lane & 3);
    a_myseq = lds_addr(&sh.xseq[w][lane]);
    p_pub = (lds_int_p)&sh.ctl_pub[0];
    p_u = (lds_f2_p)&sh.ctl_rec[0][jr][0];
    a_rec0 = ((lane & 12) == 0) ? lds_addr(&sh.rec[0][jr][row]) : lds_addr(&sh.dump[w][lane]);
    int left = spin_budget_init(a.spin_budget, a.T, a.fault_wave == w + 1);
    if constexpr (GATED) {
      const uint32_t a_go = lds_addr(&sh.gate_open[0]);
      while (lds_peek(a_go) == 0 && --left > 0) __builtin_amdgcn_s_sleep(1);
      const volatile float *gs = sh.gstate;
      sv = gs[3 + row];
    } else {
      sv = a.state[3 + row];
    }
    while (__builtin_amdgcn_readfirstlane(*p_pub) < 1 && --left > 0) __builtin_amdgcn_s_sleep(1);
    budget = left;
    un = p_u[0];
    asm volatile("" : "+v"(un));
  }
  __device__ __forceinline__ void put_record(const int t)
  {
    asm volatile("ds_write_b32 %0, %1" ::"v"(a_rec0 + (uint32_t)(t & (kGRing - 1)) * kRecStride), "v"(sv) : "memory");
    lds_publish(a_myseq, t + 1);
  }
  __device__ __forceinline__ f32x2 open(const int t)
  {
    const f32x2 u = un;
    put_record(t);
    return u;
  }
  __device__ __forceinline__ void request(const int tn)
  {
    sn = (tn & (kGRing - 1)) * kSlotF2;
// ... 110 lines not shown
```

autorally_amd/csrc/mppi_abi.hip:

```cpp
#include "abi_internal.hpp"

using namespace mppi;
using namespace mppi_abi;


namespace mppi {
thread_local hipEvent_t tl_kernel_start = nullptr, tl_kernel_stop = nullptr;
}

namespace mppi_abi {

int fail(mppi_handle *h, int code, const char *what, hipError_t e)
{
  if (h) {
    h->err = what;
    if (e != hipSuccess) {
      h->err += ": ";
      h->err += hipGetErrorString(e);
    }
  }
  return code;
}

int own_stream(mppi_handle *h)
// ... 139 lines not shown
  }
  const size_t KT2 = (size_t)h->K * h->T * 2;
#define CR(call)                                                        \
  do {                                                                  \
    hipError_t e__ = (call);                                            \
    if (e__ != hipSuccess) {                                            \
      fprintf(stderr, "mppi_create: %s: %s\n", #call, hipGetErrorString(e__)); \
      free_all(h);                                                      \
      return MPPI_ERR_HIP;                                              \
    }                                                                   \
  } while (0)
  CR(hipStreamCreateWithFlags(&h->stream, hipStreamNonBlocking));
  {
    int lo = 0, hi = 0;
    const char *e = getenv("MPPI_GSTREAM_PRIO");
    if ((e == nullptr || atoi(e) != 0) && hipDeviceGetStreamPriorityRange(&lo, &hi) == hipSuccess && lo != hi)
      CR(hipStreamCreateWithPriority(&h->gstream, hipStreamNonBlocking, lo));
    else
      CR(hipStreamCreateWithFlags(&h->gstream, hipStreamNonBlocking));
  }
  CR(hipEventCreateWithFlags(&h->ev_gen, hipEventDisableTiming));
  CR(hipEventCreate(&h->ev_gt[0]));
  CR(hipEventCreate(&h->ev_gt[1]));
  CR(hipEventCreateWithFlags(&h->ev_s1, hipEventDisableTiming));
  CR(hipEventCreateWithFlags(&h->ev_arm, hipEventDisableTiming));
  h->n_slots = std::max(1, cfg->num_iters);
  CR(hipMalloc(&h->d_in_buf[0], sizeof(float) * (2 * (size_t)h->T + 4)));
  CR(hipMalloc(&h->d_in_buf[1], sizeof(float) * (2 * (size_t)h->T + 4)));
  h->d_in = h->d_in_buf[0];
  CR(hipMalloc(&h->d_scal, sizeof(float) * 4));
  CR(hipMalloc(&h->d_noise, sizeof(float) * KT2 * (size_t)h->n_slots));
  CR(hipMalloc(&h->d_gen[0], sizeof(float) * KT2));
  CR(hipMalloc(&h->d_gen[1], sizeof(float) * KT2));
  h->v_buf = h->d_gen[0];
  h->gen_async = (size_t)h->K * (size_t)h->T >= ((size_t)1 << 20);
  CR(hipMalloc(&h->d_ug, sizeof(unsigned long long) * 2 * (size_t)h->T));
  CR(hipMemset(h->d_ug, 0, sizeof(unsigned long long) * 2 * (size_t)h->T));
  CR(hipMalloc(&h->d_counter, sizeof(unsigned) * (1 + (size_t)h->T)));
  CR(hipMemset(h->d_counter, 0, sizeof(unsigned) * (1 + (size_t)h->T)));
  if (h->K > 4096) {
    const size_t part_bytes = sizeof(unsigned long long) * (size_t)h->T * (h->K / 64) * 2;
    CR(hipMalloc(&h->d_part, part_bytes));
    CR(hipMemset(h->d_part, 0, part_bytes));
    CR(hipMalloc(&h->d_gx, sizeof(unsigned long long) * kTailExchangeGranules));
    CR(hipMemset(h->d_gx, 0, sizeof(unsigned long long) * kTailExchangeGranules));
  }
  CR(hipMalloc(&h->d_min_cost, sizeof(unsigned long long) * kMinCostLines * kMinCostStride));
  CR(hipMemset(h->d_min_cost, 0xFF, sizeof(unsigned long long) * kMinCostLines * kMinCostStride));
  if (const char *e = getenv("MPPI_MIN_COST")) h->use_min_cost = atoi(e) != 0;
  if (const char *e = getenv("MPPI_MIN_COST_TAG")) h->min_cost_tag = (unsigned)strtoul(e, nullptr, 0);
  CR(hipMalloc(&h->d_stage, sizeof(float) * KT2));
  CR(hipMalloc(&h->d_costs, sizeof(float) * h->K));
  CR(hipMalloc(&h->d_w, sizeof(float) * h->K));
  CR(hipMalloc(&h->d_costs_alt, sizeof(float) * h->K));
  CR(hipMalloc(&h->d_w_alt, sizeof(float) * h->K));
  CR(hipMalloc(&h->d_theta, sizeof(float) * h->net.num_params));
  CR(hipMalloc(&h->d_theta_s, sizeof(float) * h->net.num_params));
  if (h->mfma_ok)
    CR(hipMalloc(&h->d_wpack, sizeof(float) * 64 * (size_t)mfma_pack_floats_per_lane(h->hidden, h->n_hidden)));
  if (h->mfma_ok && row_variant_supported(h->hidden, h->n_hidden)) CR(hipMalloc(&h->d_rowpack, sizeof(float) * (size_t)row_pack_floats()));
  if (basis) CR(hipMalloc(&h->d_bfrowpack, sizeof(float) * (size_t)bf_row_pack_floats()));
  if (h->mfma_ok && row64_variant_supported(h->hidden, h->n_hidden))
    CR(hipMalloc(&h->d_row64pack, sizeof(float) * (size_t)row64_pack_floats(h->n_hidden)));
  if (h->mfma_ok && m44_variant_supported(h->hidden, h->n_hidden))
    CR(hipMalloc(&h->d_m44pack, sizeof(float) * (size_t)m44_pack_floats(h->n_hidden)));
  if (!basis && lds44_supported(h->net)) CR(hipMalloc(&h->d_lds44pack, sizeof(float) * (size_t)lds44_pack_floats(h->net)));
  if (!basis && lds128_supported(h->net)) {
    h->lds128_bytes = sizeof(float) * (size_t)lds128_pack_floats(h->net);
    CR(hipMalloc(&h->d_lds128pack, h->lds128_bytes));
  }
  if (!basis && lds16_supported(h->net)) {
    h->lds16_bytes = sizeof(float) * (size_t)lds16_pack_floats(h->net);
    CR(hipMalloc(&h->d_lds16pack, h->lds16_bytes));
  }
  if (!basis) CR(hipMalloc(&h->d_tracepack, sizeof(float) * h->net.num_params));
  h->trace_chunk = std::min(h->K, kTraceChunk);
  CR(hipMalloc(&h->d_trace, sizeof(float) * (size_t)h->trace_chunk * ((size_t)h->T * (kStateDim + kControlDim + 1) + 2)));
  CR(hipHostMalloc(&h->h_trace_ks, sizeof(int) * (size_t)h->trace_chunk, hipHostMallocMapped));
  {
    void *dp = nullptr;
    CR(hipHostGetDevicePointer(&dp, h->h_trace_ks, 0));
    h->d_trace_ks = static_cast<int *>(dp);
  }
  CR(hipMalloc(&h->d_rng[0], sizeof(uint32_t) * 6 * h->K));
  CR(hipMalloc(&h->d_rng[1], sizeof(uint32_t) * 6 * h->K));
  CR(hipMalloc(&h->d_jump, sizeof(uint32_t) * 18 * h->noise_C));
  CR(hipMalloc(&h->d_sub, sizeof(uint32_t) * 18 * 32));
  CR(hipMalloc(&h->d_one, sizeof(uint32_t) * 18 * 64));
  CR(hipHostMalloc(&h->h_in, sizeof(float) * (2 * (size_t)h->T + 4), hipHostMallocDefault));
  CR(hipHostMalloc(&h->h_res, sizeof(float) * 4 * ((size_t)h->T + 2), hipHostMallocMapped));
  memset(h->h_res, 0, sizeof(float) * 4 * ((size_t)h->T + 2));
  {
    void *dp = nullptr;
    CR(hipHostGetDevicePointer(&dp, h->h_res, 0));
    h->d_res_map = static_cast<float *>(dp);
  }
  {
    const size_t gate_bytes = sizeof(float) * 2 * gate_block_stride(h->T);
    void *gp = nullptr;
    if (prop.isLargeBar && hipExtMallocWithFlags(&gp, gate_bytes, hipDeviceMallocFinegrained) == hipSuccess && gp != nullptr) {
      h->gate_cpu = h->d_gate = static_cast<unsigned *>(gp);
      h->gate_bar = true;
      CR(hipMemset(gp, 0, gate_bytes));
    } else {
      (void)hipGetLastError();
      CR(hipHostMalloc(&gp, gate_bytes, hipHostMallocMapped));
      h->gate_cpu = static_cast<unsigned *>(gp);
      memset(gp, 0, gate_bytes);
      void *dp = nullptr;
      CR(hipHostGetDevicePointer(&dp, gp, 0));
      h->d_gate = static_cast<unsigned *>(dp);
    }
  }
  CR(hipMalloc(&h->d_invt, sizeof(double) * (size_t)h->T));
  {
    std::vector<double> invt((size_t)h->T, 0.0);
    for (int t = 1; t < h->T; t++) invt[t] = 1.0 / (double)t;
    CR(hipMemcpy(h->d_invt, invt.data(), sizeof(double) * (size_t)h->T, hipMemcpyHostToDevice));
  }
  CR(hipMemset(h->d_scal, 0, sizeof(float) * 4));
  h->ev.resize(cfg->num_iters);
  for (auto &s : h->ev)
    for (auto &e : s.e) CR(hipEventCreate(&e));
#undef CR
  int rc = upload_rng_tables(h);
  if (rc == MPPI_OK) rc = seed_device(h, cfg->seed, 0);
  if (rc == MPPI_OK && hipStreamSynchronize(h->stream) != hipSuccess) rc = MPPI_ERR_HIP;
  if (rc != MPPI_OK) {
    fprintf(stderr, "mppi_create: rng setup failed: %s\n", h->err.c_str());
    free_all(h);
    return rc;
  }
  *out = h;
  return MPPI_OK;
}

int mppi_destroy(mppi_handle *h)
{
  if (!h) return MPPI_ERR_INVALID;
  (void)hipSetDevice(h->cfg.device);
  (void)solve_ahead_disarm(h);
  if (h->order_stream && h->order_stream != h->stream) (void)hipStreamSynchronize(h->order_stream);
  if (h->gstream) (void)hipStreamSynchronize(h->gstream);
  if (h->stream) (void)hipStreamSynchronize(h->stream);
  free_all(h);
  return MPPI_OK;
}

int mppi_set_bf_params(mppi_handle *h, const float *W, size_t n)
{
  if (!h || !W) return MPPI_ERR_INVALID;
  DISARM(h);
  if (!h->basis) return fail(h, MPPI_ERR_STATE, "handle was created with a network (n_layers != 0)");
  if (n != (size_t)(4 * kNumBfs)) return fail(h, MPPI_ERR_INVALID, "W size != 4 * 25");
  HIPCHK(h, hipSetDevice(h->cfg.device));
  OWN(h);
  HIPCHK(h, hipStreamSynchronize(h->stream));
  h->theta.assign(W, W + n);
  HIPCHK(h, hipMemcpy(h->d_theta, W, n * sizeof(float), hipMemcpyHostToDevice));
  {
    const std::vector<float> pk = pack_bf_row_weights(h->theta);
    HIPCHK(h, hipMemcpy(h->d_bfrowpack, pk.data(), pk.size() * sizeof(float), hipMemcpyHostToDevice));
  }
  h->have_nn = true;
  return MPPI_OK;
}

int mppi_set_nn_params(mppi_handle *h, const float *theta, size_t n)
{
// ... 454 lines not shown
```

autorally_amd/csrc/mppi_device.hpp:

```cpp
#pragma once

#include <hip/hip_runtime.h>
#include <stdint.h>

namespace mppi {

constexpr int kStateDim = 7;
constexpr int kControlDim = 2;
constexpr int kNetIn = 6;
constexpr int kNetOut = 4;
constexpr int kRolloutsPerWave = 16;

struct CostArgs {
  float desired_speed, speed_coeff, track_coeff, max_slip_ang, slip_penalty, track_slop;
  float crash_coeff, steering_coeff, throttle_coeff, boundary_threshold;
  float crash_cost_discounted;
  int l1_cost;
  float r_c1[3], r_c2[3], trs[3];
  int affine;
  int need_control_cost;
  int map_w, map_h;
  const float *map;
};

struct RolloutArgs {
  float state[kStateDim];
  const float *U;
  float *noise;
  float *costs;
  const float *wpack;
  const double *inv_t;
  const uint32_t *rng_in;
  uint32_t *rng_out;
  int inline_noise;
  int K, T, opt_delay, k99;
  float nu[2], u_lo[2], u_hi[2], dt;
  int negate_yaw_der;
  int spin_budget, fault_wave;
  const unsigned *gate;
  unsigned gate_seq;
  unsigned gate_ticks;
  unsigned long long *min_cost;
  unsigned min_cost_tag;
  CostArgs cost;
};
constexpr int kGateReplicas = 8;
constexpr int kGateUOffset = 16 * kGateReplicas;
inline int gate_hist_offset(int T) { return kGateUOffset + 2 * T; }
inline size_t gate_block_floats(int T) { return (size_t)gate_hist_offset(T) + 4; }
constexpr unsigned kGateCancel = 0x80000000u;

constexpr int kMinCostLines = 8, kMinCostStride = 16;
__device__ __forceinline__ unsigned cost_order_bits(float x)
{
  const unsigned b = __float_as_uint(x);
  return b ^ ((b >> 31) ? 0xFFFFFFFFu : 0x80000000u);
}
__device__ __forceinline__ float cost_from_order_bits(unsigned o)
{
  return __uint_as_float(o ^ ((o >> 31) ? 0x80000000u : 0xFFFFFFFFu));
}
template <int CTRL>
__device__ __forceinline__ float wave_dpp(float v)
{
  return __int_as_float(__builtin_amdgcn_update_dpp(0, __float_as_int(v), CTRL, 0xF, 0xF, true));
}
template <bool MIN>
__device__ __forceinline__ float wave_reduce(float v)
{
#define MPPI_RED(A, B) (MIN ? fminf((A), (B)) : (A) + (B))
  v = MPPI_RED(v, wave_dpp<0xB1>(v));
  v = MPPI_RED(v, wave_dpp<0x4E>(v));
  v = MPPI_RED(v, wave_dpp<0x141>(v));
  v = MPPI_RED(v, wave_dpp<0x140>(v));
  const auto x = __builtin_amdgcn_permlane16_swap(__float_as_uint(v), __float_as_uint(v), false, false);
  v = MPPI_RED(__uint_as_float(x[0]), __uint_as_float(x[1]));
  const auto y = __builtin_amdgcn_permlane32_swap(__float_as_uint(v), __float_as_uint(v), false, false);
  v = MPPI_RED(__uint_as_float(y[0]), __uint_as_float(y[1]));
#undef MPPI_RED
  return v;
}
__device__ __forceinline__ void publish_min_cost(const RolloutArgs &a, const float mine)
{
  if (a.min_cost == nullptr) return;
  const float m = wave_reduce<true>((mine == mine) ? mine : INFINITY);
  if ((threadIdx.x & 63) == 0 && m < INFINITY) {
    const unsigned long long key = ((unsigned long long)(~a.min_cost_tag) << 32) | cost_order_bits(m);
    (void)__hip_atomic_fetch_min(a.min_cost + (blockIdx.x % kMinCostLines) * kMinCostStride, key, __ATOMIC_RELAXED, __HIP_MEMORY_SCOPE_AGENT);
  }
}
__device__ __forceinline__ bool load_min_cost(const unsigned long long *min_cost, const unsigned tag, float &beta)
{
  if (min_cost == nullptr) return false;
  unsigned long long k[kMinCostLines];
#pragma unroll
  for (int i = 0; i < kMinCostLines; i++) k[i] = __hip_atomic_load(min_cost + i * kMinCostStride, __ATOMIC_RELAXED, __HIP_MEMORY_SCOPE_AGENT);
  unsigned long long best = k[0];
#pragma unroll
  for (int i = 1; i < kMinCostLines; i++) best = (k[i] < best) ? k[i] : best;
  beta = cost_from_order_bits((unsigned)best);
  return (unsigned)(best >> 32) == ~tag;
}

constexpr int kMaxBatch = 4;
template <int NB>
struct QuadBatchArgsT {
  int n;
  RolloutArgs inst[NB];
};
using QuadBatchArgs = QuadBatchArgsT<kMaxBatch>;
template <int NB>
inline QuadBatchArgsT<NB> batch_args_prefix(const QuadBatchArgs &b)
{
  QuadBatchArgsT<NB> s;
  s.n = b.n;
  for (int i = 0; i < NB; i++) s.inst[i] = b.inst[i];
  return s;
}
static_assert(kMaxBatch == 4, "MPPI_BATCH_DISPATCH");
#define MPPI_BATCH_DISPATCH(NB, B, BODY)     \
  do {                                      \
    if constexpr ((NB) == 2) {              \
      if (blockIdx.y == 0) BODY((B).inst[0]); \
      else BODY((B).inst[1]);               \
    } else {                                \
      switch ((int)blockIdx.y) {            \
        case 0: BODY((B).inst[0]); break;   \
        case 1: BODY((B).inst[1]); break;   \
// ... 224 lines not shown
```

autorally_amd/csrc/mppi_kernels.hpp:

```cpp
#pragma once
#include "mppi_device.hpp"

#include <hip/hip_ext.h>
#include <type_traits>

namespace mppi {

extern thread_local hipEvent_t tl_kernel_start, tl_kernel_stop;
#define MPPI_LAUNCH_ROLLOUT(kern, grid, block, lds, stream, ...)                                                   \
  do {                                                                                                             \
    if (::mppi::tl_kernel_start != nullptr)                                                                        \
      hipExtLaunchKernelGGL(kern, grid, block, lds, stream, ::mppi::tl_kernel_start, ::mppi::tl_kernel_stop, 0,    \
                            __VA_ARGS__);                                                                          \
    else                                                                                                           \
      hipLaunchKernelGGL(kern, grid, block, lds, stream, __VA_ARGS__);                                             \
  } while (0)

template <class F>
inline hipError_t dispatch_cost_flags(bool affine, bool ctrl, F &&f)
{
  if (affine && !ctrl) return f(std::true_type{}, std::false_type{});
  if (affine && ctrl) return f(std::true_type{}, std::true_type{});
  if (!affine && !ctrl) return f(std::false_type{}, std::false_type{});
  return f(std::false_type{}, std::true_type{});
// ... 157 lines not shown
constexpr int kGlb44AheadLds = MPPI_GLB44_AHEAD_LDS;
constexpr int kGlb44BiasQuads = 7;
bool glb44_supported(const NetDesc &net);
int glb44_pack_floats(const NetDesc &net);
size_t glb44_head_bytes(const NetDesc &net);
int glb44_stream_quads(const NetDesc &net);
int glb44_resident_quads(const NetDesc &net, int cap);
size_t glb44_lds_bytes(const NetDesc &net, int cap);
size_t glb44_lds_limit();
hipError_t launch_rollout_glb44(const NetDesc &net, const RolloutArgs &a, int cap, hipStream_t stream);
hipError_t launch_rollout_glb44_batch(const NetDesc &net, const QuadBatchArgs &b, int cap, hipStream_t stream);

hipError_t launch_rollout_bf(const RolloutArgs &a, int waves, hipStream_t stream);
hipError_t launch_rollout_bf_batch(const QuadBatchArgs &b, hipStream_t stream);
hipError_t launch_dynamics_bf(const float *W, const float *states, const float *controls, float *ders, int n,
                              hipStream_t stream);

constexpr int kBfRowSlots = 7, kBfRowPackEntries = 6;
constexpr unsigned kBfRowPlain = 1u, kBfRowBigOnly = 1u << 8, kBfRowUsed = 1u << 16, kBfRowDouble = 1u << 24;
int bf_row_pack_floats();
hipError_t launch_rollout_bf_row(const RolloutArgs &a, hipStream_t stream);
hipError_t launch_rollout_bf_row_batch(const QuadBatchArgs &b, hipStream_t stream);

struct TraceArgs {
  float state[kStateDim];
  const float *V;
  const int *ks;
  const float *wimg;
  const double *inv_t;
  float *states;
  float *controls;
  float *step_costs;
  float *costs;
  int *first_crash;
  int n, K, T;
  float nu[2], u_lo[2], u_hi[2], dt;
  int negate_yaw_der;
  CostArgs cost;
};
bool trace_image_in_lds(const NetDesc &net);
hipError_t launch_rollout_trace(const NetDesc &net, const TraceArgs &a, hipStream_t stream);
hipError_t launch_rollout_trace_bf(const TraceArgs &a, hipStream_t stream);

struct TailLaunch {
  const float *costs, *V, *hist;
  float *U, *w, *scal, *res, *slid;
  unsigned *counter;
  int K, T, last_iter, slide_stride;
  unsigned seq;
  float gamma, init0, init1;
  unsigned long long *ug = nullptr;
  int no_device_copy = 0;
  float *hist_out = nullptr;
  unsigned long long *gx = nullptr, *gpart = nullptr;
  unsigned epoch = 0, poll_ticks = 0;
  int fault = 0;
  const unsigned long long *min_cost = nullptr;
  unsigned min_cost_tag = 0;
};
bool tail_is_stream(int K);
constexpr int kTailExchangeGranules = 3 * 64 + 32 * 16 + 32 * 64;
hipError_t launch_solve_tail(const TailLaunch &l, hipStream_t stream);
hipError_t launch_solve_tail_batch(const TailLaunch *l, int n, hipStream_t stream);
size_t solve_tail_fleet_arg_bytes();
void fill_solve_tail_fleet(void *dst, const TailLaunch *l, int n);
hipError_t launch_solve_tail_fleet(const TailLaunch *l, int n, const void *d_args, hipStream_t stream);
hipError_t launch_debug_cost(const CostArgs &c, float x, float y, float heading, int width_m, int height_m,
                             int ppm, float *out, hipStream_t stream);
hipError_t launch_slide(float *in, int T, int stride, float init0, float init1, hipStream_t stream);
hipError_t launch_kt_to_tk(const float *src, float *dst, int K, int T, hipStream_t stream);
hipError_t launch_tk_to_kt(const float *src, float *dst, int K, int T, hipStream_t stream);

hipError_t launch_noise(const uint32_t *rng_in, uint32_t *rng_out, const uint32_t *jump, int K, int T,
                        int L, int C, float *eps, hipStream_t stream);
struct NoiseFleetDesc {
  const uint32_t *rng_in;
  uint32_t *rng_out;
  const uint32_t *jump;
  float *eps;
  int K, T, L, C;
};
hipError_t launch_noise_fleet(const NoiseFleetDesc *h_desc, const NoiseFleetDesc *d_desc, int n, hipStream_t stream);
hipError_t launch_noise_init(uint32_t *rng, int K, const uint32_t base[6], const uint32_t *sub,
                             int sub_bits, const uint32_t *one, uint64_t offset, hipStream_t stream);

struct DdpFleetArgs {
  const float *theta;
  const float *wimg;
  const float *in;
  float *out, *work;
  int T, negate_yaw_der;
  int img_lds;
  float dt;
  float u_lo[2], u_hi[2], Q[7], R[2], Qf[7];
  NetDesc net;
};
__host__ __device__ inline int ddp_fleet_hidden(const NetDesc &net)
{
  int s = 0;
  for (int l = 1; l + 1 < net.n_layers; l++) s += net.layers[l];
  return s;
}
inline size_t ddp_fleet_in_floats(int T) { return 7 + (size_t)9 * T; }
inline size_t ddp_fleet_out_floats(int T) { return (size_t)26 * T + 2; }
inline size_t ddp_fleet_work_floats(int T, const NetDesc &net) { return (size_t)T * (7 + 2 + 2 + 72 + ddp_fleet_hidden(net)); }
bool ddp_fleet_image_in_lds(const NetDesc &net);
hipError_t launch_ddp_fleet(const DdpFleetArgs *h_inst, const DdpFleetArgs *d_inst, int n, hipStream_t stream);
hipError_t launch_device_tanhf(const float *in, float *out, size_t n, hipStream_t stream);

struct NominalFleetArgs {
  const float *wimg;
  const float *in;
  float *out;
  int T, negate_yaw_der;
  int img_lds;
  float dt;
  float u_lo[2], u_hi[2];
  NetDesc net;
};
inline size_t nominal_fleet_in_floats(int T) { return 7 + (size_t)2 * T; }
inline size_t nominal_fleet_out_floats(int T) { return (size_t)9 * T; }
bool nominal_fleet_image_in_lds(const NetDesc &net);
hipError_t launch_nominal_fleet(const NominalFleetArgs *h_inst, const NominalFleetArgs *d_inst, int n, hipStream_t stream);

}
```

autorally_amd/csrc/noise_mrg32k3a.hip:

```cpp
#include "noise_device.hpp"
#include "mppi_kernels.hpp"

namespace mppi {

__device__ __forceinline__ void noise_body(const int block, const uint32_t *__restrict__ rng_in, uint32_t *__restrict__ rng_out,
                                           const uint32_t *__restrict__ jump, const int K, const int T, const int L, const int C,
                                           float2 *__restrict__ eps)
{
  const int tid = block * blockDim.x + threadIdx.x;
  if (tid >= K * C) return;
  const int c = tid / K;
  const int k = tid - c * K;
  Mrg g;
  g.s10 = rng_in[k]; g.s11 = rng_in[K + k]; g.s12 = rng_in[2 * K + k];
  g.s20 = rng_in[3 * K + k]; g.s21 = rng_in[4 * K + k]; g.s22 = rng_in[5 * K + k];
  if (c > 0) {
    const uint32_t *J = jump + (size_t)c * 18;
    mat3_vec_m1(J, g.s10, g.s11, g.s12);
    mat3_vec_m2(J + 9, g.s20, g.s21, g.s22);
  }
  const int t0 = c * L, t1 = min(T, t0 + L);
  for (int t = t0; t < t1; t++) {
    eps[(size_t)t * K + k] = noise_pair(g);
  }
  if (c == C - 1) {
    rng_out[k] = g.s10; rng_out[K + k] = g.s11; rng_out[2 * K + k] = g.s12;
    rng_out[3 * K + k] = g.s20; rng_out[4 * K + k] = g.s21; rng_out[5 * K + k] = g.s22;
  }
}

__global__ __launch_bounds__(256) void noise_kernel(const uint32_t *__restrict__ rng_in,
                                                    uint32_t *__restrict__ rng_out,
                                                    const uint32_t *__restrict__ jump, int K, int T,
                                                    int L, int C, float2 *__restrict__ eps)
{
  noise_body((int)blockIdx.x, rng_in, rng_out, jump, K, T, L, C, eps);
}

__global__ __launch_bounds__(256) void noise_fleet_kernel(const NoiseFleetDesc *__restrict__ desc, const int n)
{
  if ((int)blockIdx.y >= n) return;
  const NoiseFleetDesc &d = desc[blockIdx.y];
  noise_body((int)blockIdx.x, load_global_ptr(d.rng_in), load_global_ptr(d.rng_out), load_global_ptr(d.jump), d.K, d.T, d.L, d.C,
             reinterpret_cast<float2 *>(load_global_ptr(d.eps)));
}

__global__ void noise_init_kernel(uint32_t *__restrict__ rng, int K, Mrg base,
                                  const uint32_t *__restrict__ sub, int sub_bits,
                                  const uint32_t *__restrict__ one, uint64_t offset)
{
  const int k = blockIdx.x * blockDim.x + threadIdx.x;
  if (k >= K) return;
  Mrg g = base;
  for (int b = 0; b < sub_bits; b++)
    if ((k >> b) & 1) {
      mat3_vec_m1(sub + b * 18, g.s10, g.s11, g.s12);
      mat3_vec_m2(sub + b * 18 + 9, g.s20, g.s21, g.s22);
    }
  for (int b = 0; b < 64; b++)
    if ((offset >> b) & 1ULL) {
      mat3_vec_m1(one + b * 18, g.s10, g.s11, g.s12);
      mat3_vec_m2(one + b * 18 + 9, g.s20, g.s21, g.s22);
    }
  rng[k] = g.s10; rng[K + k] = g.s11; rng[2 * K + k] = g.s12;
  rng[3 * K + k] = g.s20; rng[4 * K + k] = g.s21; rng[5 * K + k] = g.s22;
}

hipError_t launch_noise(const uint32_t *rng_in, uint32_t *rng_out, const uint32_t *jump, int K, int T,
                        int L, int C, float *eps, hipStream_t stream)
{
  const int total = K * C;
  hipLaunchKernelGGL(noise_kernel, dim3((total + 255) / 256), dim3(256), 0, stream, rng_in, rng_out,
                     jump, K, T, L, C, reinterpret_cast<float2 *>(eps));
  return hipGetLastError();
}

hipError_t launch_noise_fleet(const NoiseFleetDesc *h_desc, const NoiseFleetDesc *d_desc, int n, hipStream_t stream)
{
  if (!h_desc || !d_desc || n < 1 || n > kMaxFleet) return hipErrorInvalidValue;
  int blocks = 0;
  for (int i = 0; i < n; i++) {
    if (h_desc[i].K % 64 != 0) return hipErrorInvalidValue;
    const int b = (h_desc[i].K * h_desc[i].C + 255) / 256;
    blocks = b > blocks ? b : blocks;
  }
  if (blocks == 0) return hipSuccess;
  hipLaunchKernelGGL(noise_fleet_kernel, dim3(blocks, n), dim3(256), 0, stream, d_desc, n);
  return hipGetLastError();
}

hipError_t launch_noise_init(uint32_t *rng, int K, const uint32_t base[6], const uint32_t *sub,
                             int sub_bits, const uint32_t *one, uint64_t offset, hipStream_t stream)
{
  Mrg b{base[0], base[1], base[2], base[3], base[4], base[5]};
  hipLaunchKernelGGL(noise_init_kernel, dim3((K + 255) / 256), dim3(256), 0, stream, rng, K, b, sub,
                     sub_bits, one, offset);
  return hipGetLastError();
}

}
```

autorally_amd/csrc/rollout_bf_row.hip:

```cpp
#include "bf_row_device.hpp"

namespace mppi {

struct BfRowShared {
  static constexpr int NW = 4;
  static constexpr int NSW = 1;
  static constexpr bool kRecByAll = true;
  static constexpr int kR = 16;
  int xseq[NW][64];
  float rec[kGRing][kRolloutsPerWave][4];
  int cost_done[64];
  float ctl_b1[kGRing][64];
  float ctl_rec[kGRing][kRolloutsPerWave][4];
  int ctl_pub[64];
  float tex[kGRing][kRolloutsPerWave][2];
  int pose_pub[64];
  float eps[kGRing][kRolloutsPerWave][2];
  int rng_pub[64];
  int fail[4];
  int fin[8];
  float gstate[8];
  int gate_open[8];
  float dump[NW][64];
};

template <bool GATED>
__device__ __forceinline__ void bf_row_dynamics(const RolloutArgs &a, BfRowShared &sh, const int w)
{
  const int lane = threadIdx.x & 63;
  const int r = lane >> 4, p = lane & 15, j = p >> 2, y = p & 3;
  const int jr = 4 * w + r;
  const int T = a.T;
  BfRowLane L;
  bf_row_load(a.wpack, p, L);

  const uint32_t a_myseq = lds_addr(&sh.xseq[w][lane]);
  typedef const volatile int __attribute__((address_space(3))) *lds_int_p;
  typedef const volatile f32x2 __attribute__((address_space(3))) *lds_f2_p;
  const lds_int_p p_pub = (lds_int_p)&sh.ctl_pub[0];
  const lds_f2_p p_u = (lds_f2_p)&sh.ctl_rec[0][jr][0];
  constexpr int kSlotF2 = kRolloutsPerWave * 2;
  const uint32_t a_rec0 = (y == 0) ? lds_addr(&sh.rec[0][jr][j]) : lds_addr(&sh.dump[w][lane]);
  const uint32_t rec_stride = (y == 0) ? (uint32_t)(sizeof(float) * kRolloutsPerWave * 4) : 0u;

  int budget = spin_budget_init(a.spin_budget, T, a.fault_wave == w + 1);
  float s3, s4, s5, s6;
  if constexpr (GATED) {
    const uint32_t a_go = lds_addr(&sh.gate_open[0]);
    while (lds_peek(a_go) == 0 && --budget > 0) __builtin_amdgcn_s_sleep(1);
    const volatile float *gs = sh.gstate;
    s3 = gs[3]; s4 = gs[4]; s5 = gs[5]; s6 = gs[6];
  } else {
    s3 = a.state[3]; s4 = a.state[4]; s5 = a.state[5]; s6 = a.state[6];
  }
  float sj = bf_sel4(j, s3, s4, s5, s6);
  int cp = 0;
  while ((cp = __builtin_amdgcn_readfirstlane(*p_pub)) < 1 && --budget > 0) __builtin_amdgcn_s_sleep(1);
  f32x2 un = p_u[0];

  for (int t = 0; t < T; t++) {
    const f32x2 u = un;
    asm volatile("ds_write_b32 %0, %1" ::"v"(a_rec0 + (uint32_t)(t & (kGRing - 1)) * rec_stride), "v"(sj) : "memory");
    lds_publish(a_myseq, t + 1);
    if (t == T - 1) break;
    const lds_f2_p pu = p_u + ((t + 1) & (kGRing - 1)) * kSlotF2;
    const int cp_v = *p_pub;
    un = *pu;
    const float d = bf_row_deriv(L, y, s3, s4, s5, s6, u.x, u.y);
    sj = fmaf(d, a.dt, sj);
    s3 = bf_row_bc<0>(sj); s4 = bf_row_bc<4>(sj); s5 = bf_row_bc<8>(sj); s6 = bf_row_bc<12>(sj);
    cp = __builtin_amdgcn_readfirstlane(cp_v);
    const int want = t + 2;
    if (__builtin_expect(cp < want, 0)) {
      while (cp < want && --budget > 0) {
        cp = __builtin_amdgcn_readfirstlane(*p_pub);
        un = *pu;
      }
    }
  }
  spin_finish(budget, lds_addr(&sh.fail[0]), lds_addr(&sh.fin[w]));
}

template <bool AFFINE, bool CTRL, bool GATED>
__device__ __forceinline__ void bf_row_group(const RolloutArgs &a, BfRowShared &sh)
{
  using SH = BfRowShared;
  using R = GroupRoles<SH>;
  const int lane = threadIdx.x & 63;
  const int role = __builtin_amdgcn_readfirstlane(threadIdx.x >> 6);
  MrgHalf g0{0, 0, 0};
  if (role == R::kRng) g0 = group_rng_load<SH>(a);
// ... 116 lines not shown
```

autorally_amd/csrc/rollout_oct.hip:

```cpp
#include "mfma_net.hpp"
#include "group_roles.hpp"
#include "mppi_kernels.hpp"

namespace mppi {

template <int H, int NHID>
struct OctShared {
  static constexpr int NW = 4;
  static constexpr int NSW = NHID;
  static constexpr int kR = 16;
  static constexpr bool kRecByAll = false;
  float xb[2][NW][64][4];
  int xseq[NW][64];
  float rec[kGRing][kRolloutsPerWave][4];
  int cost_done[64];
  float ctl_b1[kGRing][64];
  float ctl_rec[kGRing][kRolloutsPerWave][4];
  int ctl_pub[64];
  float tex[kGRing][kRolloutsPerWave][2];
  int pose_pub[64];
  float eps[kGRing][kRolloutsPerWave][2];
  int rng_pub[64];
  int fail[4];
  int fin[8];
};

__device__ __forceinline__ void oct_poll(const uint32_t (&a_seq)[3], const uint32_t (&a_x)[3], int &f, f32x4 (&oth)[3])
{
  int f0, f1, f2;
  asm volatile(
      "ds_read_b32 %0, %6\n\tds_read_b128 %3, %9\n\t"
      "ds_read_b32 %1, %7\n\tds_read_b128 %4, %10\n\t"
      "ds_read_b32 %2, %8\n\tds_read_b128 %5, %11\n\t"
      "s_waitcnt lgkmcnt(0)"
      : "=&v"(f0), "=&v"(f1), "=&v"(f2), "=&v"(oth[0]), "=&v"(oth[1]), "=&v"(oth[2])
      : "v"(a_seq[0]), "v"(a_seq[1]), "v"(a_seq[2]), "v"(a_x[0]), "v"(a_x[1]), "v"(a_x[2])
      : "memory");
  f = __builtin_amdgcn_readfirstlane(min(min(f0, f1), f2));
}

template <int H, int NHID, int W>
__device__ __forceinline__ void oct_dynamics(const RolloutArgs &a, OctShared<H, NHID> &sh)
{
  using N = MfmaNet<H, NHID>;
  constexpr int MT = N::MT, KSH = N::KSH, NSW = NHID;
  static_assert(MT == 4, "one M tile per dynamics wave: 64-wide hidden layers");
  const int lane = threadIdx.x & 63;
  const int j = lane & 15, g = lane >> 4;
  const int T = a.T;

  float A0[2], B0[4], AH[(NHID - 1) * KSH + 1], Bh[(NHID - 1) * 4 + 1], AL[KSH], BL[4];
  A0[0] = a.wpack[(W * 2 + 0) * 64 + lane];
  A0[1] = a.wpack[(W * 2 + 1) * 64 + lane];
#pragma unroll
  for (int r = 0; r < 4; r++) B0[r] = a.wpack[(N::nA + W * 4 + r) * 64 + lane] * kTanhScale;
#pragma unroll
  for (int l = 1; l < NHID; l++) {
#pragma unroll
    for (int s = 0; s < KSH; s++)
      AH[(l - 1) * KSH + s] = a.wpack[(N::nA0 + (l - 1) * N::nAH + W * KSH + s) * 64 + lane];
#pragma unroll
    for (int r = 0; r < 4; r++) Bh[(l - 1) * 4 + r] = a.wpack[(N::nA + l * MT * 4 + W * 4 + r) * 64 + lane] * kTanhScale;
  }
#pragma unroll
  for (int s = 0; s < KSH; s++) AL[s] = a.wpack[(N::nA0 + (NHID - 1) * N::nAH + s) * 64 + lane];
#pragma unroll
  for (int r = 0; r < 4; r++) BL[r] = a.wpack[(N::nA + NHID * MT * 4 + r) * 64 + lane];

  const uint32_t a_myseq = lds_addr(&sh.xseq[W][lane]);
  const uint32_t a_xmine = lds_addr(&sh.xb[0][W][lane][0]);
  uint32_t a_seq[3], a_xo[3];
#pragma unroll
  for (int i = 0; i < 3; i++) {
    a_seq[i] = lds_addr(&sh.xseq[(W + 1 + i) & 3][0]);
    a_xo[i] = lds_addr(&sh.xb[0][(W + 1 + i) & 3][lane][0]);
  }
  const uint32_t a_pub = lds_addr(&sh.ctl_pub[0]);
  const uint32_t a_cd = lds_addr(&sh.cost_done[0]);
  constexpr uint32_t kXbParity = 4 * 64 * 4 * 4;

  typedef const volatile int __attribute__((address_space(3))) *lds_int_p;
  typedef const volatile float __attribute__((address_space(3))) *lds_float_p;
  const lds_int_p p_pub = (lds_int_p)&sh.ctl_pub[0];
  const lds_int_p p_cd = (lds_int_p)&sh.cost_done[0];
  const lds_float_p p_b1 = (lds_float_p)&sh.ctl_b1[0][lane];

  float s3 = a.state[3], s4 = a.state[4], s5 = a.state[5], s6 = a.state[6];
  int budget = spin_budget_init(a.spin_budget, T, a.fault_wave == W + 1);
  while (lds_peek(a_pub) < 1 && --budget > 0) __builtin_amdgcn_s_sleep(1);
  float b1_next = sh.ctl_b1[0][lane];
  asm volatile("" : "+v"(b1_next));
  int cp_v = 0, cd_v = 0;
  float b1n_v = 0.0f;
// ... 141 lines not shown
```

autorally_amd/csrc/rollout_row.hip:

```cpp
#include "group_roles.hpp"
#include "mppi_kernels.hpp"

namespace mppi {

#ifdef MPPI_ROW_STAMPS
__device__ unsigned long long g_row_stamps[16];
#define RSTAMP(i)                                                                                         \
  do {                                                                                                    \
    if (blockIdx.x == 0 && (threadIdx.x & 63) == 0) {                                                     \
      unsigned long long t__;                                                                             \
      asm volatile("s_memtime %0\n\ts_waitcnt lgkmcnt(0)" : "=s"(t__)::"memory");                           \
      g_row_stamps[i] = t__;                                                                              \
    }                                                                                                     \
  } while (0)
#else
#define RSTAMP(i) do { } while (0)
#endif

template <int H>
struct RowShared {
  static constexpr int NW = 4;
  static constexpr int NSW = 1;
  static constexpr bool kRecByAll = true;
  static constexpr int kR = 16;
  int xseq[NW][64];
  float rec[kGRing][kRolloutsPerWave][4];
  int cost_done[64];
  float ctl_b1[kGRing][64];
  float ctl_rec[kGRing][kRolloutsPerWave][4];
  int ctl_pub[64];
  float tex[kGRing][kRolloutsPerWave][2];
  int pose_pub[64];
  float eps[kGRing][kRolloutsPerWave][2];
  int rng_pub[64];
  int fail[4];
  int fin[8];
  float gstate[8];
  int gate_open[8];
  float dump[NW][64 * 2 + (kGRing - 1) * kRolloutsPerWave * 4];
};

template <int H, bool TREE>
struct RowWeights {
  f32x2 w1[kNetIn], w2[H], w3[TREE ? 4 : H];
  f32x2 b1s, b2s, b3;
};

constexpr int kRowPackEntries = 40;
template <int H, bool TREE>
__device__ __forceinline__ void row_load(const float *rowpack, int p, RowWeights<H, TREE> &W)
{
  static_assert(H == 32, "entry layout of pack_row_weights");
  const float4 *pk = reinterpret_cast<const float4 *>(rowpack) + p;
#pragma unroll
  for (int i = 0; i < 3; i++) {
    const float4 v = pk[i * 16];
    W.w1[2 * i] = f32x2{v.x, v.y};
    W.w1[2 * i + 1] = f32x2{v.z, v.w};
  }
#pragma unroll
  for (int i = 0; i < H / 2; i++) {
    const float4 v = pk[(3 + i) * 16];
    W.w2[2 * i] = f32x2{v.x, v.y};
    W.w2[2 * i + 1] = f32x2{v.z, v.w};
    if constexpr (!TREE) {
      const float4 u = pk[(3 + H / 2 + i) * 16];
      W.w3[2 * i] = f32x2{u.x, u.y};
      W.w3[2 * i + 1] = f32x2{u.z, u.w};
    }
  }
  const float4 b = pk[35 * 16];
  W.b1s = f32x2{b.x, b.y};
  W.b2s = f32x2{b.z, b.w};
  if constexpr (TREE) {
    const float4 u = pk[37 * 16], v = pk[38 * 16], c = pk[39 * 16];
    W.w3[0] = f32x2{u.x, u.y};
    W.w3[1] = f32x2{u.z, u.w};
    W.w3[2] = f32x2{v.x, v.y};
    W.w3[3] = f32x2{v.z, v.w};
    W.b3 = f32x2{c.x, c.y};
  } else {
    const float4 c = pk[36 * 16];
    W.b3 = f32x2{c.x, c.y};
  }
}

template <int Q>
__device__ __forceinline__ float row_bc(float a)
{
  return __int_as_float(__builtin_amdgcn_mov_dpp(__float_as_int(a), 0x150 + Q, 0xF, 0xF, false));
}
template <int Q>
__device__ __forceinline__ f32x2 row_bc2(f32x2 a)
{
  return __builtin_bit_cast(f32x2, (long long)__builtin_amdgcn_mov_dpp(__builtin_bit_cast(long long, a), 0x150 + Q, 0xF, 0xF, false));
}
template <int Q>
__device__ __forceinline__ void row_dot_step(f32x2 &z, f32x2 &b, const f32x2 *w, f32x2 a)
{
  z = __builtin_elementwise_fma(w[2 * Q], f32x2{b.x, b.x}, z);
  __builtin_amdgcn_sched_barrier(0);
  const f32x2 bn = row_bc2<(Q + 1 < 16 ? Q + 1 : 15)>(a);
  __builtin_amdgcn_sched_barrier(0);
  z = __builtin_elementwise_fma(w[2 * Q + 1], f32x2{b.y, b.y}, z);
  __builtin_amdgcn_sched_barrier(0);
  b = bn;
}
__device__ __forceinline__ f32x2 row_dot_bc(const f32x2 *w, f32x2 a)
{
  f32x2 z = {0.0f, 0.0f};
  f32x2 b = row_bc2<0>(a);
  __builtin_amdgcn_sched_barrier(0);
#define RD4(Q) row_dot_step<Q>(z, b, w, a); row_dot_step<Q + 1>(z, b, w, a); row_dot_step<Q + 2>(z, b, w, a); row_dot_step<Q + 3>(z, b, w, a);
  RD4(0) RD4(4) RD4(8) RD4(12)
#undef RD4
  return z;
// ... 297 lines not shown
```

autorally_amd/csrc/rollout_row64.hip:

```cpp
#include "group_roles.hpp"
#include "mppi_kernels.hpp"

namespace mppi {

constexpr int kH64 = 64;
constexpr int kPF = 8;

template <int NHID, int R>
struct Row64Shared {
  static constexpr int NW = R / 2;
  static constexpr int NSW = 1;
  static constexpr int kR = R;
  static constexpr bool kRecByAll = true;
  f32x2 wl[NHID - 1][kH64][32];
  int xseq[NW][64];
  float rec[kGRing][kRolloutsPerWave][4];
  int cost_done[64];
  float ctl_b1[kGRing][64];
  float ctl_rec[kGRing][kRolloutsPerWave][4];
  int ctl_pub[64];
  float tex[kGRing][kRolloutsPerWave][2];
  int pose_pub[64];
  float eps[kGRing][kRolloutsPerWave][2];
  int rng_pub[64];
  int fail[4];
  int fin[16];
  float dump[NW][64 * kGRing];
};

template <int NHID>
struct Row64Regs {
  f32x2 w1[kNetIn];
  f32x2 bs[NHID];
  f32x2 q[2], p[2];
  float bo;
};
template <int NHID>
constexpr int row64_reg_entries() { return 3 + (NHID + 1) / 2 + 3; }

template <int NHID>
__device__ __forceinline__ void row64_load(const float *pack, int g, Row64Regs<NHID> &W)
{
  constexpr int NB = (NHID + 1) / 2;
  const float4 *pk = reinterpret_cast<const float4 *>(pack) + g;
#pragma unroll
  for (int i = 0; i < 3; i++) {
    const float4 v = pk[i * 32];
    W.w1[2 * i] = f32x2{v.x, v.y};
    W.w1[2 * i + 1] = f32x2{v.z, v.w};
  }
#pragma unroll
  for (int i = 0; i < NB; i++) {
    const float4 v = pk[(3 + i) * 32];
    W.bs[2 * i] = f32x2{v.x, v.y};
    if (2 * i + 1 < NHID) W.bs[2 * i + 1] = f32x2{v.z, v.w};
  }
  const float4 u = pk[(3 + NB) * 32], v = pk[(4 + NB) * 32], c = pk[(5 + NB) * 32];
  W.q[0] = f32x2{u.x, u.y};
  W.q[1] = f32x2{u.z, u.w};
  W.p[0] = f32x2{v.x, v.y};
  W.p[1] = f32x2{v.z, v.w};
  W.bo = c.x;
}

template <int Q>
__device__ __forceinline__ float r64_bc(float a)
{
  return __int_as_float(__builtin_amdgcn_mov_dpp(__float_as_int(a), 0x150 + Q, 0xF, 0xF, false));
}
__device__ __forceinline__ void r64_rows(float a, float &lo, float &up)
{
  auto x = __builtin_amdgcn_permlane16_swap(__float_as_uint(a), __float_as_uint(a), false, false);
  lo = __uint_as_float(x[0]);
  up = __uint_as_float(x[1]);
}
template <int P>
__device__ __forceinline__ f32x2 r64_pair(f32x2 L, f32x2 U)
{
  const f32x2 src = (P < 16) ? L : U;
  return __builtin_bit_cast(f32x2, (long long)__builtin_amdgcn_mov_dpp(__builtin_bit_cast(long long, src), 0x150 + (P & 15), 0xF, 0xF, false));
}
typedef const volatile f32x2 __attribute__((address_space(3))) *r64_lds_p;
template <int P>
__device__ __forceinline__ void r64_step(f32x2 &z, f32x2 &b, f32x2 *ring, r64_lds_p base, f32x2 L, f32x2 U)
{
  constexpr int K = 2 * P;
  const f32x2 w0 = ring[K % kPF];
  if constexpr (K + kPF < kH64) ring[K % kPF] = base[(K + kPF) * 32];
  z = __builtin_elementwise_fma(w0, f32x2{b.x, b.x}, z);
  __builtin_amdgcn_sched_barrier(0);
  const f32x2 bn = r64_pair<(P + 1 < kH64 / 2 ? P + 1 : kH64 / 2 - 1)>(L, U);
  const f32x2 w1 = ring[(K + 1) % kPF];
  if constexpr (K + 1 + kPF < kH64) ring[(K + 1) % kPF] = base[(K + 1 + kPF) * 32];
  __builtin_amdgcn_sched_barrier(0);
  z = __builtin_elementwise_fma(w1, f32x2{b.y, b.y}, z);
// ... 208 lines not shown
```

Measured before the change: 107.1 million.

## Split inline MRG32k3a noise generation across two half-waves using jump-ahead

For row-form rollouts with T up to 128, the RNG wave now uses both 32-lane halves. Each half generates noise for half the horizon, starting from a mid-horizon stream state that a jump matrix precomputes. The full-horizon eps buffer is kept in LDS so the serial RNG chain that feeds the rollout is roughly halved. This costs a larger LDS eps array, twice the RNG state storage, an extra jump computation per step, and an occasional noise_mid kernel launch when the mid state is stale.

```diff
diff --git a/autorally_amd/build.py b/autorally_amd/build.py
--- a/autorally_amd/build.py
+++ b/autorally_amd/build.py
@@ -9,7 +9,7 @@
 LIB = os.path.join(HERE, "libmppi_hip.so")
 SOURCES = ["mppi_abi.hip", "abi_forms.hip", "abi_pack.hip", "abi_solve.hip", "abi_host.hip", "abi_trace.hip", "rollout_mfma.hip", "rollout_multi.hip", "rollout_oct.hip", "rollout_row.hip", "rollout_row64.hip", "rollout_m44.hip", "rollout_lds44.hip", "rollout_lds128.hip", "rollout_lds16.hip", "rollout_fleet16.hip", "rollout_fleet_multi.hip", "rollout_glb16.hip", "rollout_glb44.hip", "rollout_valu.hip", "rollout_trace.hip", "ddp_fleet.hip", "nominal_fleet.hip", "solve_kernels.hip",
            "noise_mrg32k3a.hip", "rollout_bf.hip", "rollout_bf_row.hip", "ddp_feedback.cpp"]
-HEADERS = ["abi_internal.hpp", "mppi_device.hpp", "mfma_net.hpp", "group_roles.hpp", "m44_core.hpp", "m44_group.hpp", "multi_group.hpp", "wave16_step.hpp", "wave16_image.hpp", "mppi_kernels.hpp", "noise_device.hpp", "ddp_feedback.hpp", "basis_funcs.hpp", "bf_device.hpp", "bf_row_device.hpp", "host_net.hpp", "tanhf_vec.hpp", "tanhf_scalar.hpp", "ddp_fleet_device.hpp", os.path.join("..", "..", "include", "mppi_hip.h")]
+HEADERS = ["abi_internal.hpp", "mppi_device.hpp", "mfma_net.hpp", "group_roles.hpp", "m44_core.hpp", "m44_group.hpp", "multi_group.hpp", "wave16_step.hpp", "wave16_image.hpp", "mppi_kernels.hpp", "noise_device.hpp", "mrg_jump.hpp", "ddp_feedback.hpp", "basis_funcs.hpp", "bf_device.hpp", "bf_row_device.hpp", "host_net.hpp", "tanhf_vec.hpp", "tanhf_scalar.hpp", "ddp_fleet_device.hpp", os.path.join("..", "..", "include", "mppi_hip.h")]
 FLAGS = ["--offload-arch=gfx950", "-O3", "-ffp-contract=off", "-fPIC", "-std=c++17", "-Wall",
          "-Wno-unused-function", "-mllvm", "-amdgpu-mfma-vgpr-form", "-Xarch_host", "-mavx2", "-Xarch_host", "-mfma"]
 
diff --git a/autorally_amd/csrc/abi_internal.hpp b/autorally_amd/csrc/abi_internal.hpp
--- a/autorally_amd/csrc/abi_internal.hpp
+++ b/autorally_amd/csrc/abi_internal.hpp
@@ -157,6 +157,7 @@
   bool valu_reg_ok = false;
   double *d_invt = nullptr;
   uint32_t *d_rng[2] = {nullptr, nullptr};
+  bool rng_mid_ok[2] = {false, false};
   uint32_t *d_jump = nullptr, *d_sub = nullptr, *d_one = nullptr;
   int rng_cur = 0;
   int noise_L = 1, noise_C = 1;
diff --git a/autorally_amd/csrc/abi_pack.hip b/autorally_amd/csrc/abi_pack.hip
--- a/autorally_amd/csrc/abi_pack.hip
+++ b/autorally_amd/csrc/abi_pack.hip
@@ -1,43 +1,10 @@
 #include "abi_internal.hpp"
+#include "mrg_jump.hpp"
 
 using namespace mppi;
 using namespace mppi_abi;
 
 namespace mppi_abi {
-
-constexpr uint64_t M1 = 4294967087ULL, M2 = 4294944443ULL;
-
-struct Mat3 {
-  uint32_t a[9];
-};
-Mat3 mat_mul(const Mat3 &A, const Mat3 &B, uint64_t m)
-{
-  Mat3 R;
-  for (int i = 0; i < 3; i++)
-    for (int j = 0; j < 3; j++) {
-      uint64_t acc = 0;
-      for (int k = 0; k < 3; k++) acc = (acc + (uint64_t)A.a[3 * i + k] * B.a[3 * k + j] % m) % m;
-      R.a[3 * i + j] = (uint32_t)acc;
-    }
-  return R;
-}
-Mat3 mat_identity()
-{
-  Mat3 R{{1, 0, 0, 0, 1, 0, 0, 0, 1}};
-  return R;
-}
-Mat3 mat_pow(Mat3 A, uint64_t e, uint64_t m)
-{
-  Mat3 R = mat_identity();
-  while (e) {
-    if (e & 1) R = mat_mul(R, A, m);
-    A = mat_mul(A, A, m);
-    e >>= 1;
-  }
-  return R;
-}
-Mat3 base_A1() { return Mat3{{0, 1, 0, 0, 0, 1, (uint32_t)(M1 - 810728ULL), 1403580u, 0}}; }
-Mat3 base_A2() { return Mat3{{0, 1, 0, 0, 0, 1, (uint32_t)(M2 - 1370589ULL), 0, 527612u}}; }
 
 int compute_k99(int K)
 {
@@ -407,15 +374,17 @@
   }
   int sub_bits = 0;
   while ((1LL << sub_bits) < (long long)h->K) sub_bits++;
-  HIPCHK(h, launch_noise_init(h->d_rng[0], h->K, base, h->d_sub, sub_bits, h->d_one, offset, h->stream));
+  HIPCHK(h, launch_noise_init(h->d_rng[0], h->K, base, h->d_sub, sub_bits, h->d_one, offset, h->d_jump + 18 * (size_t)h->noise_C, h->stream));
   h->rng_cur = 0;
+  h->rng_mid_ok[0] = true;
+  h->rng_mid_ok[1] = false;
   h->cfg.seed = seed;
   return MPPI_OK;
 }
 
 int upload_rng_tables(mppi_handle *h)
 {
-  std::vector<uint32_t> sub(32 * 18), one(64 * 18), jump((size_t)h->noise_C * 18);
+  std::vector<uint32_t> sub(32 * 18), one(64 * 18), jump(((size_t)h->noise_C + 1) * 18);
   Mat3 a1 = base_A1(), a2 = base_A2();
   for (int b = 0; b < 64; b++) {
     memcpy(&one[(size_t)b * 18], a1.a, 36);
@@ -442,6 +411,7 @@
     c1 = mat_mul(j1, c1, M1);
     c2 = mat_mul(j2, c2, M2);
   }
+  rng_split_jump(h->T, &jump[(size_t)h->noise_C * 18]);
   HIPCHK(h, hipMemcpy(h->d_sub, sub.data(), sub.size() * 4, hipMemcpyHostToDevice));
   HIPCHK(h, hipMemcpy(h->d_one, one.data(), one.size() * 4, hipMemcpyHostToDevice));
   HIPCHK(h, hipMemcpy(h->d_jump, jump.data(), jump.size() * 4, hipMemcpyHostToDevice));
diff --git a/autorally_amd/csrc/abi_solve.hip b/autorally_amd/csrc/abi_solve.hip
--- a/autorally_amd/csrc/abi_solve.hip
+++ b/autorally_amd/csrc/abi_solve.hip
@@ -159,6 +159,7 @@
   a.negate_yaw_der = (h->cfg.negate_yaw_der || f == Form::BfRow) ? 1 : 0;
   a.rng_in = nullptr;
   a.rng_out = nullptr;
+  a.rng_jump = nullptr;
   a.inline_noise = 0;
   a.gate = nullptr;
   a.gate_seq = 0;
@@ -242,6 +243,7 @@
     h->gen_timed = true;
   }
   h->rng_cur = 1 - h->rng_cur;
+  h->rng_mid_ok[h->rng_cur] = false;
   HIPCHK(h, hipEventRecord(h->ev_gen, h->gstream));
   return MPPI_OK;
 }
@@ -254,6 +256,7 @@
     HIPCHK(h, launch_noise(h->d_rng[h->rng_cur], h->d_rng[1 - h->rng_cur], h->d_jump, h->K, h->T, h->noise_L,
                            h->noise_C, dst, h->stream));
     h->rng_cur = 1 - h->rng_cur;
+    h->rng_mid_ok[h->rng_cur] = false;
     *buf_out = dst;
     return MPPI_OK;
   }
@@ -299,12 +302,20 @@
   if (++h->tail_epoch == 0) h->tail_epoch = 1;
 }
 
-static void use_inline_noise(mppi_handle *h, RolloutArgs &a)
-{
+static int use_inline_noise(mppi_handle *h, RolloutArgs &a, hipStream_t stream)
+{
+  const bool split = form_is_row(form_of(h)) && h->T <= kRngSplitMaxT;
+  if (split && !h->rng_mid_ok[h->rng_cur]) {
+    HIPCHK(h, launch_noise_mid(h->d_rng[h->rng_cur], h->K, h->d_jump + 18 * (size_t)h->noise_C, stream));
+    h->rng_mid_ok[h->rng_cur] = true;
+  }
   a.inline_noise = 1;
   a.rng_in = h->d_rng[h->rng_cur];
   a.rng_out = h->d_rng[1 - h->rng_cur];
+  a.rng_jump = h->d_jump + 18 * (size_t)h->noise_C;
   h->rng_cur = 1 - h->rng_cur;
+  h->rng_mid_ok[h->rng_cur] = split;
+  return MPPI_OK;
 }
 
 static int hand_over(mppi_handle *h, hipStream_t batch)
@@ -531,7 +542,10 @@
     fill_rollout_args(h, state, noise, a);
     rc = tag_min_cost(h, a, h->stream);
     if (rc) return rc;
-    if (inline_noise) use_inline_noise(h, a);
+    if (inline_noise) {
+      rc = use_inline_noise(h, a, h->stream);
+      if (rc) return rc;
+    }
 #ifdef MPPI_HOSTPROF
     HP(1, hp_t0);
     const auto hp_t1 = std::chrono::steady_clock::now();
@@ -669,7 +683,10 @@
     l.no_device_copy = 1;
     l.slid = nullptr;
   }
-  if (kind == 1) use_inline_noise(h, a);
+  if (kind == 1) {
+    rc = use_inline_noise(h, a, stream);
+    if (rc) return rc;
+  }
   next_tail_epoch(h);
   l.epoch = h->tail_epoch;
   mark_armed(h, kind, noise, stream, max_wait_s, publish_only);
@@ -946,6 +963,7 @@
         noise = h->d_gen[h->gen_cur];
         nd[i] = NoiseFleetDesc{h->d_rng[h->rng_cur], h->d_rng[1 - h->rng_cur], h->d_jump, noise, h->K, h->T, h->noise_L, h->noise_C};
         h->rng_cur = 1 - h->rng_cur;
+        h->rng_mid_ok[h->rng_cur] = false;
       }
       h->v_buf = noise;
       fill_rollout_args(h, states + (size_t)MPPI_STATE_DIM * i, noise, ra[i]);
@@ -1115,7 +1133,8 @@
       RolloutArgs &a = qb.inst[i];
       fill_rollout_args(h, states + (size_t)MPPI_STATE_DIM * i, noise, a);
       if (int trc = tag_min_cost(h, a, S)) return trc;
-      if (!explicit_noise) use_inline_noise(h, a);
+      if (!explicit_noise)
+        if (int nrc = use_inline_noise(h, a, S)) return nrc;
       tl[i] = tail_launch(h, noise, last);
       if (last) h->slid_valid = wants_slid_copy(h);
     }
@@ -1264,7 +1283,10 @@
   h->v_buf = noise;
   RolloutArgs a;
   fill_rollout_args(h, state, noise, a);
-  if (inline_noise) use_inline_noise(h, a);
+  if (inline_noise) {
+    rc = use_inline_noise(h, a, h->stream);
+    if (rc) return rc;
+  }
   rc = launch_rollout(h, a);
   if (rc) return rc;
   note_solve_state(h, state, false);
diff --git a/autorally_amd/csrc/group_roles.hpp b/autorally_amd/csrc/group_roles.hpp
--- a/autorally_amd/csrc/group_roles.hpp
+++ b/autorally_amd/csrc/group_roles.hpp
@@ -41,6 +41,8 @@
   return (uint32_t)x;
 }
 template <class SH>
+__device__ __forceinline__ bool rng_split(const RolloutArgs &a) { return SH::kRngSplit && a.T <= kRngSplitMaxT; }
+template <class SH>
 __device__ __forceinline__ MrgHalf group_rng_load(const RolloutArgs &a)
 {
   const int lane = threadIdx.x & 63;
@@ -48,10 +50,37 @@
   const int k = (int)blockIdx.x * SH::kR + j;
   const int K = a.K;
   MrgHalf g{0, 0, 0};
-  if (a.inline_noise != 0 && lane < 2 * kRolloutsPerWave) {
-    g.s0 = a.rng_in[(3 * c) * K + k]; g.s1 = a.rng_in[(3 * c + 1) * K + k]; g.s2 = a.rng_in[(3 * c + 2) * K + k];
+  if (a.inline_noise != 0 && (lane < 2 * kRolloutsPerWave || rng_split<SH>(a))) {
+    const uint32_t *in = a.rng_in + (size_t)(lane >> 5) * 6 * K;
+    g.s0 = in[(3 * c) * K + k]; g.s1 = in[(3 * c + 1) * K + k]; g.s2 = in[(3 * c + 2) * K + k];
   }
   return g;
+}
+__device__ __forceinline__ float2 rng_draw_pair(MrgHalf &g, const int c, const uint32_t A, const uint32_t Bn, const uint32_t C, const uint32_t m)
+{
+  float2 e;
+#pragma unroll
+  for (int d = 0; d < 2; d++) {
+    const uint32_t p = fold_m((uint64_t)A * (c ? g.s2 : g.s1) + (uint64_t)Bn * (m - g.s0), C, m);
+    g.s0 = g.s1; g.s1 = g.s2; g.s2 = p;
+    const uint32_t p2 = (uint32_t)__builtin_amdgcn_mov_dpp((int)p, 0xB1, 0xF, 0xF, false);
+    uint32_t z = (p >= p2) ? p - p2 : p + (uint32_t)kM1 - p2;
+    if (z == 0) z = (uint32_t)kM1;
+    const float u = (float)z * 0x1p-32f;
+    if (d == 0) e.x = u; else e.y = u;
+  }
+  return e;
+}
+__device__ __forceinline__ void rng_jump(const uint32_t *J, MrgHalf &g, const uint32_t C, const uint32_t m)
+{
+  uint32_t r[3];
+#pragma unroll
+  for (int i = 0; i < 3; i++) {
+    const uint64_t acc = (uint64_t)fold_m((uint64_t)J[3 * i] * g.s0, C, m) + fold_m((uint64_t)J[3 * i + 1] * g.s1, C, m) +
+                         fold_m((uint64_t)J[3 * i + 2] * g.s2, C, m);
+    r[i] = fold_m(acc, C, m);
+  }
+  g.s0 = r[0]; g.s1 = r[1]; g.s2 = r[2];
 }
 template <class SH, bool PRE = false>
 __device__ __forceinline__ void group_rng_wave(const RolloutArgs &a, SH &sh, const MrgHalf pre = MrgHalf{0, 0, 0})
@@ -70,27 +99,53 @@
     MrgHalf g{0, 0, 0};
     if constexpr (PRE) {
       g = pre;
-    } else if (active) {
-      g.s0 = a.rng_in[(3 * c) * K + k]; g.s1 = a.rng_in[(3 * c + 1) * K + k]; g.s2 = a.rng_in[(3 * c + 2) * K + k];
+    } else if (active || rng_split<SH>(a)) {
+      const uint32_t *in = a.rng_in + (size_t)(lane >> 5) * 6 * K;
+      g.s0 = in[(3 * c) * K + k]; g.s1 = in[(3 * c + 1) * K + k]; g.s2 = in[(3 * c + 2) * K + k];
     }
     const uint32_t a_ctl = lds_addr(&sh.ctl_pub[0]);
     const uint32_t a_mypub = lds_addr(&sh.rng_pub[lane]);
+    if (rng_split<SH>(a)) {
+      const int half = lane >> 5;
+      const int hh = (T + 1) >> 1, nlo = T - hh;
+      const int tb = half ? hh : 0;
+      for (int i = 0; i < nlo; i++) {
+#ifdef MPPI_DIAG_NORNG
+        const float2 e = make_float2(0.25f + 0.001f * (float)(tb + i), 0.5f);
+#else
+        const float2 e = rng_draw_pair(g, c, A, Bn, C, m);
+#endif
+        if (c == 0) *reinterpret_cast<float2 *>(&sh.eps[tb + i][j][0]) = e;
+        lds_publish(a_mypub, i + 1);
+      }
+      if (nlo < hh) {
+        if (half == 0) {
+#ifdef MPPI_DIAG_NORNG
+          const float2 e = make_float2(0.25f + 0.001f * (float)nlo, 0.5f);
+#else
+          const float2 e = rng_draw_pair(g, c, A, Bn, C, m);
+#endif
+          if (c == 0) *reinterpret_cast<float2 *>(&sh.eps[nlo][j][0]) = e;
+        }
+        lds_publish(a_mypub, hh);
+      }
+      if (half == 1 && (lane & 31) < 2 * SH::kR) {
+        uint32_t *out = a.rng_out;
+        out[(3 * c) * K + k] = g.s0; out[(3 * c + 1) * K + k] = g.s1; out[(3 * c + 2) * K + k] = g.s2;
+        rng_jump(a.rng_jump + 9 * c, g, C, m);
+        out += (size_t)6 * K;
+        out[(3 * c) * K + k] = g.s0; out[(3 * c + 1) * K + k] = g.s1; out[(3 * c + 2) * K + k] = g.s2;
+      }
+      spin_finish(budget, lds_addr(&sh.fail[0]), lds_addr(&sh.fin[R::kRng]));
+      return;
+    }
     int seen = 0;
     for (int t = 0; t < T; t++) {
       float2 e = make_float2(0.5f, 0.5f);
 #ifdef MPPI_DIAG_NORNG
       e = make_float2(0.25f + 0.001f * (float)t, 0.5f);
 #else
-#pragma unroll
-      for (int d = 0; d < 2; d++) {
-        const uint32_t p = fold_m((uint64_t)A * (c ? g.s2 : g.s1) + (uint64_t)Bn * (m - g.s0), C, m);
-        g.s0 = g.s1; g.s1 = g.s2; g.s2 = p;
-        const uint32_t p2 = (uint32_t)__builtin_amdgcn_mov_dpp((int)p, 0xB1, 0xF, 0xF, false);
-        uint32_t z = (p >= p2) ? p - p2 : p + (uint32_t)kM1 - p2;
-        if (z == 0) z = (uint32_t)kM1;
-        const float u = (float)z * 0x1p-32f;
-        if (d == 0) e.x = u; else e.y = u;
-      }
+      e = rng_draw_pair(g, c, A, Bn, C, m);
 #endif
       const int need = t - kGRing + 1;
       while (seen < need && --budget > 0) {
@@ -119,6 +174,8 @@
   const int k = (int)blockIdx.x * SH::kR + j;
   const int K = a.K, T = a.T;
   const bool inl = a.inline_noise != 0;
+  const bool split = rng_split<SH>(a);
+  const int hh = (T + 1) >> 1;
   float2 *const noise = reinterpret_cast<float2 *>(a.noise);
   const float2 *const Useq = reinterpret_cast<const float2 *>(a.U);
   const bool noise_free_k = (k == 0);
@@ -152,14 +209,16 @@
       if (seen_x < need_x || seen_c < need_c) __builtin_amdgcn_s_sleep(2);
     }
     if (inl) {
-      while (seen_r < tm + 1 && --budget > 0) {
+      const int need_r = !split ? tm + 1 : (t0 < hh) ? min(tm, hh - 1) + 1 : tm - hh + 1;
+      while (seen_r < need_r && --budget > 0) {
         seen_r = lds_peek(a_rng);
-        if (seen_r < tm + 1) __builtin_amdgcn_s_sleep(1);
-      }
+        if (seen_r < need_r) __builtin_amdgcn_s_sleep(1);
+      }
+      const int es = split ? tl : tl & (kGRing - 1);
 #ifdef MPPI_DIAG_NOBM
-      e = *reinterpret_cast<const float2 *>(&sh.eps[tl & (kGRing - 1)][j][0]);
-#else
-      e = box_muller(*reinterpret_cast<const float2 *>(&sh.eps[tl & (kGRing - 1)][j][0]));
+      e = *reinterpret_cast<const float2 *>(&sh.eps[es][j][0]);
+#else
+      e = box_muller(*reinterpret_cast<const float2 *>(&sh.eps[es][j][0]));
 #endif
     }
     if (live) {
diff --git a/autorally_amd/csrc/m44_group.hpp b/autorally_amd/csrc/m44_group.hpp
--- a/autorally_amd/csrc/m44_group.hpp
+++ b/autorally_amd/csrc/m44_group.hpp
@@ -9,6 +9,7 @@
   static constexpr int NW = 4;
   static constexpr int NSW = 1;
   static constexpr int kR = 16;
+  static constexpr bool kRngSplit = false;
   static constexpr bool kRecByAll = true;
   int xseq[NW][64];
   float rec[kGRing][kRolloutsPerWave][4];
diff --git a/autorally_amd/csrc/mppi_abi.hip b/autorally_amd/csrc/mppi_abi.hip
--- a/autorally_amd/csrc/mppi_abi.hip
+++ b/autorally_amd/csrc/mppi_abi.hip
@@ -245,9 +245,9 @@
     CR(hipHostGetDevicePointer(&dp, h->h_trace_ks, 0));
     h->d_trace_ks = static_cast<int *>(dp);
   }
-  CR(hipMalloc(&h->d_rng[0], sizeof(uint32_t) * 6 * h->K));
-  CR(hipMalloc(&h->d_rng[1], sizeof(uint32_t) * 6 * h->K));
-  CR(hipMalloc(&h->d_jump, sizeof(uint32_t) * 18 * h->noise_C));
+  CR(hipMalloc(&h->d_rng[0], sizeof(uint32_t) * 12 * h->K));
+  CR(hipMalloc(&h->d_rng[1], sizeof(uint32_t) * 12 * h->K));
+  CR(hipMalloc(&h->d_jump, sizeof(uint32_t) * 18 * (h->noise_C + 1)));
   CR(hipMalloc(&h->d_sub, sizeof(uint32_t) * 18 * 32));
   CR(hipMalloc(&h->d_one, sizeof(uint32_t) * 18 * 64));
   CR(hipHostMalloc(&h->h_in, sizeof(float) * (2 * (size_t)h->T + 4), hipHostMallocDefault));
diff --git a/autorally_amd/csrc/mppi_device.hpp b/autorally_amd/csrc/mppi_device.hpp
--- a/autorally_amd/csrc/mppi_device.hpp
+++ b/autorally_amd/csrc/mppi_device.hpp
@@ -32,6 +32,7 @@
   const double *inv_t;
   const uint32_t *rng_in;
   uint32_t *rng_out;
+  const uint32_t *rng_jump;
   int inline_noise;
   int K, T, opt_delay, k99;
   float nu[2], u_lo[2], u_hi[2], dt;
@@ -44,6 +45,7 @@
   unsigned min_cost_tag;
   CostArgs cost;
 };
+constexpr int kRngSplitMaxT = 128;
 constexpr int kGateReplicas = 8;
 constexpr int kGateUOffset = 16 * kGateReplicas;
 inline int gate_hist_offset(int T) { return kGateUOffset + 2 * T; }
diff --git a/autorally_amd/csrc/mppi_kernels.hpp b/autorally_amd/csrc/mppi_kernels.hpp
--- a/autorally_amd/csrc/mppi_kernels.hpp
+++ b/autorally_amd/csrc/mppi_kernels.hpp
@@ -263,7 +263,8 @@
 };
 hipError_t launch_noise_fleet(const NoiseFleetDesc *h_desc, const NoiseFleetDesc *d_desc, int n, hipStream_t stream);
 hipError_t launch_noise_init(uint32_t *rng, int K, const uint32_t base[6], const uint32_t *sub,
-                             int sub_bits, const uint32_t *one, uint64_t offset, hipStream_t stream);
+                             int sub_bits, const uint32_t *one, uint64_t offset, const uint32_t *split, hipStream_t stream);
+hipError_t launch_noise_mid(uint32_t *rng, int K, const uint32_t *split, hipStream_t stream);
 
 struct DdpFleetArgs {
   const float *theta;
diff --git a/autorally_amd/csrc/mrg_jump.hpp b/autorally_amd/csrc/mrg_jump.hpp
--- /dev/null
+++ b/autorally_amd/csrc/mrg_jump.hpp
@@ -0,0 +1,51 @@
+#pragma once
+
+#include <stdint.h>
+#include <string.h>
+
+namespace mppi_abi {
+
+constexpr uint64_t M1 = 4294967087ULL, M2 = 4294944443ULL;
+
+struct Mat3 {
+  uint32_t a[9];
+};
+inline Mat3 mat_mul(const Mat3 &A, const Mat3 &B, uint64_t m)
+{
+  Mat3 R;
+  for (int i = 0; i < 3; i++)
+    for (int j = 0; j < 3; j++) {
+      uint64_t acc = 0;
+      for (int k = 0; k < 3; k++) acc = (acc + (uint64_t)A.a[3 * i + k] * B.a[3 * k + j] % m) % m;
+      R.a[3 * i + j] = (uint32_t)acc;
+    }
+  return R;
+}
+inline Mat3 mat_identity()
+{
+  Mat3 R{{1, 0, 0, 0, 1, 0, 0, 0, 1}};
+  return R;
+}
+inline Mat3 mat_pow(Mat3 A, uint64_t e, uint64_t m)
+{
+  Mat3 R = mat_identity();
+  while (e) {
+    if (e & 1) R = mat_mul(R, A, m);
+    A = mat_mul(A, A, m);
+    e >>= 1;
+  }
+  return R;
+}
+inline Mat3 base_A1() { return Mat3{{0, 1, 0, 0, 0, 1, (uint32_t)(M1 - 810728ULL), 1403580u, 0}}; }
+inline Mat3 base_A2() { return Mat3{{0, 1, 0, 0, 0, 1, (uint32_t)(M2 - 1370589ULL), 0, 527612u}}; }
+
+inline int rng_split_steps(int T) { return (T + 1) / 2; }
+inline void rng_split_jump(int T, uint32_t out[18])
+{
+  const uint64_t draws = 2ULL * (uint64_t)rng_split_steps(T);
+  const Mat3 j1 = mat_pow(base_A1(), draws, M1), j2 = mat_pow(base_A2(), draws, M2);
+  memcpy(out, j1.a, sizeof(j1.a));
+  memcpy(out + 9, j2.a, sizeof(j2.a));
+}
+
+}
diff --git a/autorally_amd/csrc/noise_mrg32k3a.hip b/autorally_amd/csrc/noise_mrg32k3a.hip
--- a/autorally_amd/csrc/noise_mrg32k3a.hip
+++ b/autorally_amd/csrc/noise_mrg32k3a.hip
@@ -45,9 +45,25 @@
              reinterpret_cast<float2 *>(load_global_ptr(d.eps)));
 }
 
+__device__ __forceinline__ void noise_put_mid(uint32_t *__restrict__ rng, const int K, const int k, Mrg g, const uint32_t *__restrict__ split)
+{
+  mat3_vec_m1(split, g.s10, g.s11, g.s12);
+  mat3_vec_m2(split + 9, g.s20, g.s21, g.s22);
+  uint32_t *mid = rng + (size_t)6 * K;
+  mid[k] = g.s10; mid[K + k] = g.s11; mid[2 * K + k] = g.s12;
+  mid[3 * K + k] = g.s20; mid[4 * K + k] = g.s21; mid[5 * K + k] = g.s22;
+}
+__global__ void noise_mid_kernel(uint32_t *__restrict__ rng, int K, const uint32_t *__restrict__ split)
+{
+  const int k = blockIdx.x * blockDim.x + threadIdx.x;
+  if (k >= K) return;
+  const Mrg g{rng[k], rng[K + k], rng[2 * K + k], rng[3 * K + k], rng[4 * K + k], rng[5 * K + k]};
+  noise_put_mid(rng, K, k, g, split);
+}
+
 __global__ void noise_init_kernel(uint32_t *__restrict__ rng, int K, Mrg base,
                                   const uint32_t *__restrict__ sub, int sub_bits,
-                                  const uint32_t *__restrict__ one, uint64_t offset)
+                                  const uint32_t *__restrict__ one, uint64_t offset, const uint32_t *__restrict__ split)
 {
   const int k = blockIdx.x * blockDim.x + threadIdx.x;
   if (k >= K) return;
@@ -64,6 +80,7 @@
     }
   rng[k] = g.s10; rng[K + k] = g.s11; rng[2 * K + k] = g.s12;
   rng[3 * K + k] = g.s20; rng[4 * K + k] = g.s21; rng[5 * K + k] = g.s22;
+  noise_put_mid(rng, K, k, g, split);
 }
 
 hipError_t launch_noise(const uint32_t *rng_in, uint32_t *rng_out, const uint32_t *jump, int K, int T,
@@ -90,11 +107,17 @@
 }
 
 hipError_t launch_noise_init(uint32_t *rng, int K, const uint32_t base[6], const uint32_t *sub,
-                             int sub_bits, const uint32_t *one, uint64_t offset, hipStream_t stream)
+                             int sub_bits, const uint32_t *one, uint64_t offset, const uint32_t *split, hipStream_t stream)
 {
   Mrg b{base[0], base[1], base[2], base[3], base[4], base[5]};
   hipLaunchKernelGGL(noise_init_kernel, dim3((K + 255) / 256), dim3(256), 0, stream, rng, K, b, sub,
-                     sub_bits, one, offset);
+                     sub_bits, one, offset, split);
+  return hipGetLastError();
+}
+
+hipError_t launch_noise_mid(uint32_t *rng, int K, const uint32_t *split, hipStream_t stream)
+{
+  hipLaunchKernelGGL(noise_mid_kernel, dim3((K + 255) / 256), dim3(256), 0, stream, rng, K, split);
   return hipGetLastError();
 }
 
diff --git a/autorally_amd/csrc/rollout_bf_row.hip b/autorally_amd/csrc/rollout_bf_row.hip
--- a/autorally_amd/csrc/rollout_bf_row.hip
+++ b/autorally_amd/csrc/rollout_bf_row.hip
@@ -7,6 +7,7 @@
   static constexpr int NSW = 1;
   static constexpr bool kRecByAll = true;
   static constexpr int kR = 16;
+  static constexpr bool kRngSplit = false;
   int xseq[NW][64];
   float rec[kGRing][kRolloutsPerWave][4];
   int cost_done[64];
diff --git a/autorally_amd/csrc/rollout_oct.hip b/autorally_amd/csrc/rollout_oct.hip
--- a/autorally_amd/csrc/rollout_oct.hip
+++ b/autorally_amd/csrc/rollout_oct.hip
@@ -9,6 +9,7 @@
   static constexpr int NW = 4;
   static constexpr int NSW = NHID;
   static constexpr int kR = 16;
+  static constexpr bool kRngSplit = false;
   static constexpr bool kRecByAll = false;
   float xb[2][NW][64][4];
   int xseq[NW][64];
diff --git a/autorally_amd/csrc/rollout_row.hip b/autorally_amd/csrc/rollout_row.hip
--- a/autorally_amd/csrc/rollout_row.hip
+++ b/autorally_amd/csrc/rollout_row.hip
@@ -31,7 +31,8 @@
   int ctl_pub[64];
   float tex[kGRing][kRolloutsPerWave][2];
   int pose_pub[64];
-  float eps[kGRing][kRolloutsPerWave][2];
+  static constexpr bool kRngSplit = true;
+  float eps[kRngSplitMaxT][kRolloutsPerWave][2];
   int rng_pub[64];
   int fail[4];
   int fin[8];
diff --git a/autorally_amd/csrc/rollout_row64.hip b/autorally_amd/csrc/rollout_row64.hip
--- a/autorally_amd/csrc/rollout_row64.hip
+++ b/autorally_amd/csrc/rollout_row64.hip
@@ -11,6 +11,7 @@
   static constexpr int NW = R / 2;
   static constexpr int NSW = 1;
   static constexpr int kR = R;
+  static constexpr bool kRngSplit = false;
   static constexpr bool kRecByAll = true;
   f32x2 wl[NHID - 1][kH64][32];
   int xseq[NW][64];
```

New measurement: 106.3 million. No clear change (-0.7%).
